# venomouscyanide/S3GRL

Hardware: AMD Instinct MI355X
Metric: link-pair precomputes/sec (higher is better)
Workload: dtype f32; 1 GPU; pubmed_pos_k3; mode=pos, sign_k=3, num_hops=3, num_nodes=19717, features=500, graph=real topology, synthetic features (BASELINE.md §3)

## Files before the change

### s3grl_amd/csrc/s3grl_api.hip

```cpp
#include <algorithm>
#include <chrono>
#include <cstdlib>
#include <cstring>
#include <memory>

#include "s3grl_internal.hpp"

namespace s3grl {

static thread_local std::string g_last_error;
void set_last_error(const std::string& msg) { g_last_error = msg; }

Arena::~Arena() {
  for (auto& kv : free_)
    if (!carved_.count(kv.second)) (void)hipFree(kv.second);
  for (auto& kv : live_)
    if (!carved_.count(kv.first)) (void)hipFree(kv.first);
  for (auto& sl : slabs_)
    if (sl.base) (void)hipFree(sl.base);
}

s3grl_status Arena::reserve(size_t bytes) {
  if (bytes < (1u << 20) || cached_ * 2 >= bytes) return S3GRL_OK;
  if (cur_slab_ >= 0 && slabs_[cur_slab_].size - slabs_[cur_slab_].used >= bytes) return S3GRL_OK;
// ... 731 lines not shown
      g_walk.balls = g->balls;
      S3GRL_TRY(launch_count_balls(ctx, &g_walk, links_walk, L, cfg->num_hops, plus ? 1 : 0, K, partner, mirror_of,
                                   plan->n_nodes, p_nodes, n_rows, n_jobs, lvl_max, reinterpret_cast<int32_t*>(ds),
                                   st + 3 * kStatRow, stash, slot, plan->lvl, perm));
    } else {
      S3GRL_TRY(launch_count(ctx, &g_walk, links_walk, L, cfg->num_hops, plus ? 1 : 0, K, ws,
                             partner, mirror_of,
                             plan->n_nodes, p_nodes, n_rows, n_jobs, lvl_max,
                             reinterpret_cast<int32_t*>(ds), st + 3 * kStatRow, smp, stash, slot, plan->lvl, perm));
    }
  }
  if (fold) S3GRL_TRY(launch_mirror_rows(ctx, partner, L, n_rows));
  S3GRL_TRY(launch_scan3(ctx, plan->n_nodes, n_rows, n_jobs, L, plan->node_off, plan->row_ptr, plan->job_off,
                         scan_ws, ds + 1, ds + 5, ds + 9));
  const bool csr_plan = !sop2 && !(cfg->flags & S3GRL_FLAG_COUNT_ONLY) && stash != nullptr && balls &&
                        csr_mode_for(g, cfg->num_hops, K, balls, relabel && !walks && !sampling && !onehop);
  if (!plus && !csr_plan)
    S3GRL_TRY(launch_classify(ctx, g, 1, K, plan->n_nodes, p_nodes, lvl_max, L, class_count, class_list,
                              !sampling && !g->directed, e_cap, stash ? slot : 0, perm, x_cap, nullptr, true));
  S3GRL_HIP_TRY(hipMemcpyAsync(hs, ds, 56 * 8, hipMemcpyDeviceToHost, ctx->stream));
  S3GRL_HIP_TRY(hipMemcpyAsync(ctx->h_stats + 3 * kStatRow, st + 3 * kStatRow, 2 * kStatRow * sizeof(int64_t),
                               hipMemcpyDeviceToHost, ctx->stream));
  S3GRL_HIP_TRY(hipStreamSynchronize(ctx->stream));
  hs[16] = hs[9];
  hs[17] = hs[10];
  hs[18] = hs[11];
  const int err = (int)(hs[0] & 0xffffffff);
  if (err == 2) {
    set_last_error("a link has src == dst");
    return S3GRL_ERR_SELF_LINK;
  }
  if (err == 1) {
    set_last_error("a link endpoint is outside [0, num_nodes)");
    return S3GRL_ERR_INVALID_ARGUMENT;
  }
  const int64_t max_n = hs[1], max_R = hs[5];
  const int64_t tot_n = hs[16], tot_rows = hs[17], njobs = hs[18];
  const int cn_cap = ((int)std::max<int64_t>(max_R - 2, 0) + 1) * ((relabel && plus) ? 3 : 1);
  uint16_t* csr_cnt = nullptr;
  int32_t* csr_e = nullptr;
  if (csr_plan) {
    S3GRL_TRY(arena_alloc(ctx, (size_t)std::max<int64_t>(tot_n, 1), &csr_cnt, tr));
    S3GRL_TRY(arena_alloc(ctx, (size_t)L, &csr_e, tr));
    S3GRL_TRY(launch_csr_count(ctx, &g_walk, links_walk, L, cfg->num_hops, plan->n_nodes, plan->node_off, plan->lvl,
                               stash, slot, perm, csr_cnt, csr_e));
  }
  if (plus || csr_plan) {
    S3GRL_TRY(launch_classify(ctx, g, plus ? cn_cap : 1, K, plan->n_nodes, p_nodes, lvl_max, L, class_count,
                              class_list, !sampling && !g->directed, e_cap, stash ? slot : 0, perm, x_cap, csr_e,
                              !plus));
    S3GRL_HIP_TRY(hipMemcpyAsync(hs + 32, ds + 32, 24 * 8, hipMemcpyDeviceToHost, ctx->stream));
    S3GRL_HIP_TRY(hipStreamSynchronize(ctx->stream));
  }
  int32_t class_count_host[48];
  std::memcpy(class_count_host, hs + 32, sizeof(class_count_host));
  if (getenv("S3GRL_DEBUG")) {
    fprintf(stderr, "[s3grl] L=%lld max_n=%lld classes:", (long long)L, (long long)max_n);
    for (int c = 0; c < num_class_lists(); ++c) fprintf(stderr, " %d", class_count_host[c]);
    fprintf(stderr, "\n");
  }
  if (cfg->flags & S3GRL_FLAG_COUNT_ONLY) {
    plan->stats.total_nodes = stat_total(3);
    plan->stats.folded_links = hs[7];
    plan->stats.extracted_nodes = tot_n;
    plan->stats.max_nodes = max_n;
    plan->stats.total_rows = tot_rows;
    plan->stats.num_row_pairs = 0;
    plan->njobs = 0;
    plan->stats.workspace_bytes = (int64_t)ctx->arena.bytes_held();
    *out = plan.release();
    return S3GRL_OK;
  }
  plan->stats.total_nodes = stat_total(3);
  plan->stats.oriented_entries = stat_total(4);
  plan->stats.folded_links = hs[7];
  plan->stats.extracted_nodes = tot_n;
  plan->stats.max_nodes = max_n;
  plan->stats.total_rows = tot_rows;
  plan->stats.num_row_pairs = njobs;
  plan->njobs = njobs;
  {
    int32_t* hist;
    S3GRL_TRY(arena_alloc(ctx, (size_t)256, &hist, tr));
    S3GRL_TRY(arena_alloc(ctx, (size_t)std::max<int64_t>(njobs, 1), &plan->job_order, own));
    int32_t* pc = nullptr;
    int64_t* po = nullptr;
    if (perm && hub_gather) {
      S3GRL_TRY(arena_alloc(ctx, (size_t)L, &pc, tr));
      S3GRL_TRY(arena_alloc(ctx, (size_t)(L + 1), &po, tr));
    }
    S3GRL_TRY(launch_job_order(ctx, plan->n_nodes, n_jobs, plan->job_off, L, hist, plan->job_order,
                               hub_gather ? perm : nullptr, pc, po, scan_ws));
  }
  plan->hub_order = perm != nullptr && hub_gather;

  const int64_t* coef_off = nullptr;
  int64_t tot_coef = tot_n;
  if (plus) {
    int32_t* job_n;
    int64_t* co;
    S3GRL_TRY(arena_alloc(ctx, (size_t)scan_workspace_elems(njobs), &scan_ws, tr));
    S3GRL_TRY(arena_alloc(ctx, (size_t)njobs, &job_n, tr));
    S3GRL_TRY(arena_alloc(ctx, (size_t)(njobs + 1), &co, tr));
    hipLaunchKernelGGL(expand_job_n_kernel, dim3((unsigned)((L + 255) / 256)), dim3(256), 0,
                       ctx->stream, plan->n_nodes, plan->job_off, L, job_n);
    S3GRL_HIP_TRY(hipGetLastError());
    S3GRL_TRY(launch_scan_i32_to_i64(ctx, job_n, njobs, co, scan_ws));
    S3GRL_HIP_TRY(hipMemcpyAsync(hs + 20, co + njobs, 8, hipMemcpyDeviceToHost, ctx->stream));
    S3GRL_HIP_TRY(hipStreamSynchronize(ctx->stream));
    tot_coef = hs[20];
    coef_off = co;
  }
  S3GRL_TRY(ctx->arena.reserve((size_t)std::max<int64_t>(tot_n, 1) * 4 + (size_t)std::max<int64_t>(tot_coef, 1) * 8 * K +
                               (size_t)njobs * (sizeof(Job) + 12 * K + 8) + (size_t)tot_rows * 8 + (16u << 20)));
  S3GRL_TRY(arena_alloc(ctx, (size_t)std::max<int64_t>(tot_n, 1), &plan->c_ids, own));
  S3GRL_TRY(arena_alloc(ctx, (size_t)std::max<int64_t>(tot_coef, 1) * 2 * K, &plan->c_coef, own));
  S3GRL_TRY(arena_alloc(ctx, (size_t)njobs, &plan->jobs, own));
  S3GRL_TRY(arena_alloc(ctx, (size_t)njobs * K * 2, &plan->job_z, own));
  S3GRL_TRY(arena_alloc(ctx, (size_t)std::max<int64_t>(njobs * K, 1), &plan->job_lim, own));
  S3GRL_TRY(arena_alloc(ctx, (size_t)tot_rows, &plan->row_nodes, own));
  int seg_shift = kSplitSegShift;
  if (const char* e = getenv("S3GRL_SPLIT_SEG_SHIFT")) seg_shift = std::min(20, std::max(4, atoi(e)));
  int split_t = kSplitThreshold;
  if (const char* e = getenv("S3GRL_SPLIT_T")) split_t = std::max(0, atoi(e));
  if (split_t > 0) split_t = std::max(split_t, 1 << seg_shift);
  if (max_n <= split_t) split_t = 0;
  plan->split_t = split_t;
  plan->seg_shift = seg_shift;
  S3GRL_TRY(record(ctx, 1));
  unsigned long long* tot = reinterpret_cast<unsigned long long*>(st);
  const LinkOut lo{plan->node_off, plan->row_ptr, plan->job_off, coef_off, mirror_of, plan->c_ids, plan->c_coef,
                    plan->jobs, plan->job_z, plan->job_lim, plan->row_nodes, plan->lvl, tot, tot + kStatRow,
                    tot + 2 * kStatRow, relabel ? g->old_of_new : nullptr, split_t, seg_shift};
  S3GRL_TRY(launch_links(ctx, &g_walk, links_walk, L, class_list, class_count_host, cfg->num_hops, plus ? 1 : 0,
                         cn_cap, (cfg->flags & S3GRL_FLAG_FULL_STATS) ? 1 : 0, K, ws, p_nodes, lo, smp, stash,
                         slot, e_cap, relabel ? g->new_of_old : nullptr, x_cap, csr_cnt, csr_e, sop2 ? 1 : 0));
  if (split_t > 0) {
    int32_t* pcnt;
    S3GRL_TRY(arena_alloc(ctx, (size_t)njobs, &pcnt, tr));
    S3GRL_TRY(arena_alloc(ctx, (size_t)(njobs + 1), &plan->piece_off, own));
    S3GRL_TRY(arena_alloc(ctx, (size_t)scan_workspace_elems(njobs), &scan_ws, tr));
    S3GRL_TRY(launch_split_count(ctx, plan->jobs, njobs, seg_shift, pcnt, plan->piece_off, scan_ws));
    S3GRL_HIP_TRY(hipMemcpyAsync(hs + 21, plan->piece_off + njobs, 8, hipMemcpyDeviceToHost, ctx->stream));
  }
  S3GRL_TRY(record(ctx, 2));
  S3GRL_HIP_TRY(hipMemcpyAsync(ctx->h_stats, st, 3 * kStatRow * sizeof(int64_t), hipMemcpyDeviceToHost,
                               ctx->stream));
  S3GRL_HIP_TRY(hipMemcpyAsync(ctx->h_stats + 4 * kStatRow, st + 4 * kStatRow, 5 * kStatRow * sizeof(int64_t),
                               hipMemcpyDeviceToHost, ctx->stream));
  plan->stats.workspace_bytes = (int64_t)ctx->arena.bytes_held();
  plan->stats_pending = true;
  ctx->stats_owner = plan.get();
  if (split_t > 0 || getenv("S3GRL_DEBUG_STAMPS")) {
    S3GRL_TRY(resolve_plan_stats(ctx));
    if (split_t > 0 && hs[21] > 0) {
      const int64_t np = hs[21];
      plan->npieces = np;
      const size_t units = (size_t)(njobs + np);
      S3GRL_TRY(arena_alloc(ctx, units, &plan->gjobs, own));
      S3GRL_TRY(arena_alloc(ctx, units * K * 2, &plan->g_z, own));
      S3GRL_TRY(arena_alloc(ctx, units * K, &plan->g_lim, own));
      S3GRL_TRY(arena_alloc(ctx, units, &plan->g_order, own));
      S3GRL_TRY(arena_alloc(ctx, (size_t)np, &plan->piece_job, own));
      S3GRL_HIP_TRY(hipMemcpyAsync(plan->g_z, plan->job_z, (size_t)njobs * K * 2 * sizeof(float),
                                   hipMemcpyDeviceToDevice, ctx->stream));
      S3GRL_HIP_TRY(hipMemsetAsync(plan->g_z + (size_t)njobs * K * 2, 0, (size_t)np * K * 2 * sizeof(float), ctx->stream));
      S3GRL_TRY(launch_split_fill(ctx, plan->jobs, plan->job_lim, njobs, plan->job_order, K, seg_shift,
                                  plan->piece_off, np, plan->gjobs, plan->g_lim, plan->g_order, plan->piece_job));
    }
    if (getenv("S3GRL_DEBUG_STAMPS")) {
      S3GRL_HIP_TRY(hipMemcpy(hs + 16, ds + 16, 8 * 8, hipMemcpyDeviceToHost));
      fprintf(stderr, "[s3grl] link_kernel phase cycles (sum over workgroups): bfs %lld  P/rank %lld  "
                      "deg %lld  ops<K %lld  last op %lld  tail %lld\n",
              (long long)hs[16], (long long)hs[17], (long long)hs[18], (long long)hs[19],
              (long long)hs[20], (long long)hs[21]);
      if (csr_plan)
        fprintf(stderr, "[s3grl] link_csr_kernel phase cycles (same slots): bitmap+ranks+offsets %lld  ids+rows %lld  "
                        "columns %lld  passes %lld   links %lld, mean LDS %lld B\n",
                (long long)hs[16], (long long)hs[17], (long long)hs[18], (long long)hs[19], (long long)hs[20],
                (long long)(hs[21] / std::max<int64_t>(hs[20], 1)));
      if (x_cap)
        fprintf(stderr, "[s3grl] link_hub_kernel phase cycles (same slots): nodes %lld  ids+rows %lld  walk %lld  "
                        "small csr %lld  passes %lld  tail %lld\n",
                (long long)hs[16], (long long)hs[17], (long long)hs[18], (long long)hs[19], (long long)hs[20],
                (long long)hs[21]);
      S3GRL_HIP_TRY(hipMemcpy(hs + 24, ds + 24, 8 * 8, hipMemcpyDeviceToHost));
      fprintf(stderr, "[s3grl] link_full_kernel, big class: merge %lld  hash+ids %lld  probes %lld  "
                      "csr+sort %lld  passes %lld   links %lld, columns in HBM for %lld\n",
              (long long)hs[24], (long long)hs[25], (long long)hs[26], (long long)hs[27], (long long)hs[28],
              (long long)hs[30], (long long)hs[31]);
    }
  }
  *out = plan.release();
  return S3GRL_OK;
}

s3grl_status s3grl_context_trim(s3grl_context* ctx, int64_t* released) {
  if (!ctx) return S3GRL_ERR_INVALID_ARGUMENT;
  S3GRL_HIP_TRY(hipSetDevice(ctx->device));
  S3GRL_HIP_TRY(hipStreamSynchronize(ctx->stream));
  for (auto& st : ctx->side)
    if (st) S3GRL_HIP_TRY(hipStreamSynchronize(st));
  const size_t freed = ctx->arena.trim();
  if (released) *released = (int64_t)freed;
  return S3GRL_OK;
}

s3grl_status s3grl_plan_gather_traffic(s3grl_context* ctx, const s3grl_plan* p,
                                       const s3grl_features* f, int64_t* what) {
  if (!ctx || !p || !f || !what) return S3GRL_ERR_INVALID_ARGUMENT;
  S3GRL_HIP_TRY(hipSetDevice(ctx->device));
  for (int i = 0; i < 8; ++i) what[i] = 0;
  if (p->njobs == 0) return S3GRL_OK;
  if (f->N != p->graph->num_nodes) return S3GRL_ERR_INVALID_ARGUMENT;
  S3GRL_HIP_TRY(hipMemsetAsync(ctx->d_scalars, 0, 8 * sizeof(int64_t), ctx->stream));
  S3GRL_TRY(launch_gather_traffic(ctx, p, f, reinterpret_cast<unsigned long long*>(ctx->d_scalars)));
  S3GRL_HIP_TRY(hipMemcpyAsync(ctx->h_scalars, ctx->d_scalars, 8 * sizeof(int64_t), hipMemcpyDeviceToHost,
                               ctx->stream));
  S3GRL_HIP_TRY(hipStreamSynchronize(ctx->stream));
  for (int i = 0; i < 8; ++i) what[i] = ctx->h_scalars[i];
  return S3GRL_OK;
}

s3grl_status s3grl_plan_get_stats(const s3grl_plan* p, s3grl_plan_stats* out) {
  if (!p || !out) return S3GRL_ERR_INVALID_ARGUMENT;
  if (p->stats_pending && p->ctx->stats_owner == p) S3GRL_TRY(resolve_plan_stats(p->ctx));
  *out = p->stats;
  return S3GRL_OK;
}

s3grl_status s3grl_plan_total_rows(const s3grl_plan* p, int64_t* total_rows) {
  if (!p || !total_rows) return S3GRL_ERR_INVALID_ARGUMENT;
  *total_rows = p->stats.total_rows;
  return S3GRL_OK;
}

s3grl_status s3grl_plan_counts(const s3grl_plan* p, int64_t* what) {
  if (!p || !what) return S3GRL_ERR_INVALID_ARGUMENT;
  what[0] = p->L;
  what[1] = p->stats.total_rows;
  what[2] = p->stats.folded_links;
  what[3] = p->njobs;
  return S3GRL_OK;
}

s3grl_status s3grl_plan_link_cost(const s3grl_plan* p, float* cost) {
  if (!p || (!cost && p->L)) return S3GRL_ERR_INVALID_ARGUMENT;
  if (p->L == 0) return S3GRL_OK;
  hipLaunchKernelGGL(link_cost_kernel, dim3((unsigned)((p->L + 255) / 256)), dim3(256), 0, p->ctx->stream,
                     p->n_nodes, p->e_cap, p->x_cap, p->row_ptr, p->L, kHubCostSlope, cost);
  S3GRL_HIP_TRY(hipGetLastError());
  return S3GRL_OK;
}

s3grl_status s3grl_plan_row_ptr(const s3grl_plan* p, int64_t* row_ptr) {
  if (!p || !row_ptr) return S3GRL_ERR_INVALID_ARGUMENT;
  S3GRL_HIP_TRY(hipMemcpyAsync(row_ptr, p->row_ptr, (size_t)(p->L + 1) * 8, hipMemcpyDeviceToDevice,
                               p->ctx->stream));
  return S3GRL_OK;
}

s3grl_status s3grl_plan_row_nodes(const s3grl_plan* p, int64_t* row_nodes) {
  if (!p || (!row_nodes && p->stats.total_rows)) return S3GRL_ERR_INVALID_ARGUMENT;
  if (p->stats.total_rows)
    S3GRL_HIP_TRY(hipMemcpyAsync(row_nodes, p->row_nodes, (size_t)p->stats.total_rows * 8,
                                 hipMemcpyDeviceToDevice, p->ctx->stream));
  return S3GRL_OK;
}

s3grl_status s3grl_plan_export_subgraphs(const s3grl_plan* p, int64_t* node_ptr, int32_t* nodes,
                                         int8_t* dists) {
  if (!p || !node_ptr) return S3GRL_ERR_INVALID_ARGUMENT;
  hipStream_t st = p->ctx->stream;
  S3GRL_HIP_TRY(hipMemcpyAsync(node_ptr, p->node_off, (size_t)(p->L + 1) * 8,
                               hipMemcpyDeviceToDevice, st));
  const size_t n = (size_t)p->stats.extracted_nodes;
  if ((nodes || dists) && (p->cfg.flags & S3GRL_FLAG_COUNT_ONLY)) {
    set_last_error("a count-only plan holds sizes only (pass NULL for nodes and dists)");
    return S3GRL_ERR_INVALID_ARGUMENT;
  }
  if (nodes && n) S3GRL_HIP_TRY(hipMemcpyAsync(nodes, p->c_ids, n * 4, hipMemcpyDeviceToDevice, st));
  if (nodes && n && p->relabelled) S3GRL_TRY(launch_sort_hops(p->ctx, p, nodes));
  if (dists && n) S3GRL_TRY(launch_dists(p->ctx, p->node_off, p->lvl, p->L, dists));
  return S3GRL_OK;
}

static s3grl_status run_with(s3grl_context* ctx, const s3grl_plan* p, const s3grl_features* f,
                             float* rows) {
  if (p->cfg.flags & S3GRL_FLAG_COUNT_ONLY) {
    set_last_error("a count-only plan cannot be run");
    return S3GRL_ERR_INVALID_ARGUMENT;
  }
  if (p->njobs == 0) return S3GRL_OK;
  if (f->N != p->graph->num_nodes) {
    set_last_error("features have " + std::to_string(f->N) + " rows, the graph " +
                   std::to_string(p->graph->num_nodes) + " nodes");
    return S3GRL_ERR_INVALID_ARGUMENT;
  }
  if (ctx->profiling) S3GRL_TRY(resolve_pending_gather(ctx));
  S3GRL_TRY(record(ctx, 3));
  auto gather = [&](const GatherView& v) -> s3grl_status {
    if (f->sparse) return launch_gather_sparse(ctx, p, v, f, rows);
    if (f->packed) return launch_gather_packed(ctx, p, v, f, rows);
    return launch_gather(ctx, v, p->c_ids, p->c_coef, p->cfg.sign_k, f->dense, f->ld, f->F, rows, p->hub_order);
  };
  if (p->npieces == 0) {
    S3GRL_TRY(gather(GatherView{p->jobs, p->njobs, p->job_z, p->job_lim, p->job_order, nullptr}));
  } else {
    Transient tmp{ctx, {}};
    void* q = nullptr;
    S3GRL_TRY(ctx->arena.alloc((size_t)p->npieces * 2 * (p->cfg.sign_k + 1) * (f->F + 1) * sizeof(float), &q));
    tmp.ptrs.push_back(q);
    float* prows = static_cast<float*>(q);
    S3GRL_TRY(gather(GatherView{p->gjobs, p->njobs + p->npieces, p->g_z, p->g_lim, p->g_order, prows}));
    S3GRL_TRY(launch_combine(ctx, p, prows, f->dense, f->ld, f->F, rows));
  }
  S3GRL_TRY(record(ctx, 4));
  if (ctx->profiling) ctx->gather_pending = true;
  return S3GRL_OK;
}

s3grl_status s3grl_run_features(s3grl_context* ctx, const s3grl_plan* p, const s3grl_features* f,
                                float* rows) {
  if (!ctx || !p || !f || (p->stats.total_rows && !rows)) return S3GRL_ERR_INVALID_ARGUMENT;
  S3GRL_HIP_TRY(hipSetDevice(ctx->device));
  return run_with(ctx, p, f, rows);
}

s3grl_status s3grl_run(s3grl_context* ctx, const s3grl_plan* p, const float* X, int64_t ldx,
                       int64_t F, float* rows) {
  if (!ctx || !p) return S3GRL_ERR_INVALID_ARGUMENT;
  if (!X) {
    set_last_error("node features are None");
    return S3GRL_ERR_NO_FEATURES;
  }
  if (F <= 0 || ldx < F || (p->stats.total_rows && !rows)) return S3GRL_ERR_INVALID_ARGUMENT;
  if (p->njobs == 0) return S3GRL_OK;
  s3grl_features* f = nullptr;
  S3GRL_TRY(s3grl_features_create(ctx, X, ldx, p->graph->num_nodes, F, 1, &f));
  const s3grl_status st = run_with(ctx, p, f, rows);
  s3grl_features_destroy(f);
  return st;
}

}

S3GRL_DEFINE_TOUCH(api)
```

### s3grl_amd/csrc/s3grl_csr.hip

```cpp
#include <hip/hip_runtime.h>

#include <algorithm>
#include <cstdlib>

#include "s3grl_device.hpp"

namespace s3grl {
namespace {

constexpr int kCsrCountT = 128;
constexpr int kCsrCountUn = 4;

__global__ __launch_bounds__(kCsrCountT) void csr_count_kernel(
    const int32_t* __restrict__ indptr, const int32_t* __restrict__ indices, int W, const uint32_t* __restrict__ balls,
    const int64_t* __restrict__ links, int hops, const int32_t* __restrict__ n_nodes,
    const int64_t* __restrict__ node_off, const int32_t* __restrict__ lvl, const int32_t* __restrict__ stash, int slot,
    const int32_t* __restrict__ perm, uint16_t* __restrict__ cnt, int32_t* __restrict__ csr_e) {
  extern __shared__ uint32_t smem[];
  constexpr int T = kCsrCountT;
  uint32_t* vis = smem;
  int* sh = reinterpret_cast<int*>(vis + W);
  const int tid = threadIdx.x;
  const int l = perm ? perm[blockIdx.x] : (int)blockIdx.x;
  const int n = n_nodes[l];
  if (n == 0 || n - 2 > slot) {
    if (tid == 0) csr_e[l] = -1;
    return;
  }
  const int src = (int)links[2 * (int64_t)l], dst = (int)links[2 * (int64_t)l + 1];
  const int64_t noff = node_off[l];
  const int32_t* lv = lvl + (int64_t)l * kMaxLevels;
  const int nlev = lv[kMaxLevels - 1];
  const int walk_from = nlev - 1 == hops ? lv[hops - 1] : n;
  const uint32_t* __restrict__ bs = balls + (int64_t)src * W;
  const uint32_t* __restrict__ bd = balls + (int64_t)dst * W;
  for (int w = tid; w < W; w += T) vis[w] = bs[w] | bd[w];
  const int32_t* __restrict__ st = stash + (int64_t)l * slot;
  const int32_t* list = st + (walk_from - 2);
  int e_local = 0;
  for (int t = tid; t < walk_from; t += T) {
    const int v = t < 2 ? (t == 0 ? min(src, dst) : max(src, dst)) : st[t - 2];
    const int b = indptr[v], d = indptr[v + 1] - b;
    int c = d;
    if (v == src || v == dst) c -= sorted_contains(indices + b, d, v == src ? dst : src) ? 1 : 0;
    cnt[noff + t] = (uint16_t)c;
    e_local += c;
  }
  __syncthreads();
  walk_rows<T, 4, kCsrCountUn>(
      0, n - walk_from, list, indptr, indices, nullptr,
      [&](RowAcc& a, int v, int u, bool valid) {
        const int mp = v == src ? dst : (v == dst ? src : -1);
        a.n += (valid && test_bit(vis, u) && u != mp) ? 1 : 0;
      },
      [&](RowAcc& a, int t, int) {
        cnt[noff + walk_from + t] = (uint16_t)a.n;
        e_local += a.n;
      });
  e_local = block_sum<T>(e_local, sh);
  if (tid == 0) csr_e[l] = e_local <= 65535 ? e_local : -1;
}

template <int T>
__global__ __launch_bounds__(T) void link_csr_kernel(const CsrLinkArgs a, const int32_t* __restrict__ class_list,
                                                     const int K) {
  extern __shared__ uint32_t smem[];
  constexpr int G = 4, RPI = T / G;
  const int32_t* __restrict__ indptr = a.indptr;
  const int32_t* __restrict__ indices = a.indices;
  const LinkOut& out = a.out;
  const int tid = threadIdx.x;
  const int l = class_list[blockIdx.x];
  const int64_t noff = out.node_off[l];
  const int n = (int)(out.node_off[l + 1] - noff);
  const int e = a.csr_e[l];
  const int W = a.W;
  const int mirror = out.mirror_of ? out.mirror_of[l] : -1;
  const int64_t mrp = mirror >= 0 ? out.row_ptr[mirror] : -1;

  int32_t* cn = reinterpret_cast<int32_t*>(smem);
  int32_t* cnpos = cn + a.cn_cap;
  int* lvl_end = cnpos + a.cn_cap;
  float* zbuf = reinterpret_cast<float*>(lvl_end + kMaxLevels);
  int* sh = reinterpret_cast<int*>(zbuf + 4 * K);
  float* dtab = reinterpret_cast<float*>(sh + 32);
  uint16_t* off = reinterpret_cast<uint16_t*>(dtab + kCsrDinvTable);
  uint16_t* cols = off + ((n + 2) & ~1);
  char* ubase = reinterpret_cast<char*>(smem) +
                (((reinterpret_cast<char*>(cols + ((e + 1) & ~1)) - reinterpret_cast<char*>(smem)) + 7) & ~(size_t)7);
  uint32_t* vis = reinterpret_cast<uint32_t*>(ubase);
  uint32_t* wpre = vis + W;
  int32_t* gb = reinterpret_cast<int32_t*>(wpre + W);
  uint16_t* gdeg = reinterpret_cast<uint16_t*>(gb + n);
  uint16_t* por = gdeg + ((n + 1) & ~1);
  float2* cur = reinterpret_cast<float2*>(ubase);
  float2* nxs = cur + n;

  unsigned long long t_prev = a.dbg ? __builtin_amdgcn_s_memtime() : 0ull;
  const int src = (int)a.links[2 * (int64_t)l], dst = (int)a.links[2 * (int64_t)l + 1];
  const int pos_src = src < dst ? 0 : 1, pos_dst = 1 - pos_src;
  const int32_t* lv = out.lvl + (int64_t)l * kMaxLevels;
  const int nlev = lv[kMaxLevels - 1];
  if (tid < nlev) lvl_end[tid] = lv[tid];
  for (int d = tid; d < kCsrDinvTable; d += T) dtab[d] = d > 0 ? 1.0f / sqrtf((float)d) : 0.0f;
  {
    const uint32_t* __restrict__ bs = a.balls + (int64_t)src * W;
    const uint32_t* __restrict__ bd = a.balls + (int64_t)dst * W;
    for (int w = tid; w < W; w += T) vis[w] = bs[w] | bd[w];
  }
  __syncthreads();
  {
    const int CW = (W + T - 1) / T, CN = (n + T - 1) / T;
    const int w0 = min(tid * CW, W), w1 = min(w0 + CW, W);
    const int t0 = min(tid * CN, n), t1 = min(t0 + CN, n);
    int pop = 0, cnt = 0;
    for (int w = w0; w < w1; ++w) pop += __popc(vis[w]);
    for (int t = t0; t < t1; ++t) cnt += a.cnt[noff + t];
    int total;
    const int run = block_excl_scan<T>((pop << 16) | cnt, sh, total);
    int rp_ = run >> 16, ro = run & 0xffff;
    for (int w = w0; w < w1; ++w) {
      wpre[w] = rp_;
      rp_ += __popc(vis[w]);
    }
    for (int t = t0; t < t1; ++t) {
      off[t] = (uint16_t)ro;
      ro += a.cnt[noff + t];
    }
    if (tid == 0) off[n] = (uint16_t)(total & 0xffff);
  }
  __syncthreads();
  phase_stamp(a.dbg, 0, t_prev);
  int vol_local = 0;
  {
    const int32_t* __restrict__ st = a.stash + (int64_t)l * a.slot;
    for (int t0 = tid; t0 < n; t0 += 4 * T) {
      int v[4], b[4], en[4];
#pragma unroll
      for (int k = 0; k < 4; ++k) {
        const int t = min(t0 + k * T, n - 1);
        v[k] = t < 2 ? (t == 0 ? min(src, dst) : max(src, dst)) : st[t - 2];
      }
#pragma unroll
      for (int k = 0; k < 4; ++k) {
        b[k] = indptr[(uint32_t)v[k]];
        en[k] = indptr[(uint32_t)v[k] + 1u];
      }
#pragma unroll
      for (int k = 0; k < 4; ++k) {
        const int t = t0 + k * T;
        if (t < n) {
          out.c_ids[noff + t] = ext_id(out, v[k]);
          vol_local += en[k] - b[k];
          gb[t] = b[k];
          gdeg[t] = (uint16_t)(en[k] - b[k]);
          por[rank_of(vis, wpre, v[k])] = (uint16_t)t;
        }
      }
    }
  }
  const int64_t rp = out.row_ptr[l];
  const int R = (int)(out.row_ptr[l + 1] - rp);
  const LinkSlot ls{l, src, dst, mirror, noff, rp, mrp};
  if (a.plus && wave_id() == 0) {
    auto in_s = [&](int u) -> bool { return test_bit(vis, u); };
    const int c = common_neighbours(indptr, indices, in_s, src, dst, cn);
    sort_caller_order(cn, c, out.old_of_new, lane_id());
  }
  __syncthreads();
  for (int r = tid; r < R; r += T) {
    const int node = row_node(r, src, dst, cn);
    write_row_node(out, ls, r, node);
    if (r >= 2) cnpos[r - 2] = por[rank_of(vis, wpre, node)];
  }
  if (tid == 0)
    for (int d = 0; d < kMaxLevels; ++d) export_level(out, l, d, nlev, lvl_end[d], n);

  phase_stamp(a.dbg, 1, t_prev);
  {
    const int g = tid & (G - 1);
    const int nib_shift = (tid & 63) & ~(G - 1);
    for (int base = 0; base < n; base += 2 * RPI) {
      int c0[2], e1[2], wc[2], mp[2], nx[2];
#pragma unroll
      for (int u = 0; u < 2; ++u) {
        const int t = base + u * RPI + tid / G;
        const bool ok = t < n;
        const int b = gb[min(t, n - 1)];
        c0[u] = ok ? b + g : 0;
        e1[u] = ok ? b + (int)gdeg[min(t, n - 1)] : 0;
        wc[u] = off[min(t, n)];
        mp[u] = t == pos_src ? dst : (t == pos_dst ? src : -1);
      }
#pragma unroll
      for (int u = 0; u < 2; ++u) nx[u] = indices[(uint32_t)(c0[u] < e1[u] ? c0[u] : 0)];
      while (__any(c0[0] < e1[0] || c0[1] < e1[1])) {
#pragma unroll
        for (int u = 0; u < 2; ++u) {
          const bool valid = c0[u] < e1[u];
          const int uu = nx[u];
          const int cnx = c0[u] + G;
          uint32_t an = (uint32_t)(cnx < e1[u] ? cnx : 0);
          asm volatile("" : "+v"(an));
          nx[u] = indices[an];
          const uint32_t bit = 1u << (uu & 31);
          const uint32_t wv = vis[uu >> 5];
          const int r = (int)wpre[uu >> 5] + __popc(wv & (bit - 1u));
          const int col = por[min(r, n - 1)];
          const bool member = valid && (wv & bit) && uu != mp[u];
          const unsigned nib = (unsigned)(__ballot(member) >> nib_shift) & ((1u << G) - 1u);
          if (member) cols[wc[u] + __popc(nib & ((1u << g) - 1u))] = (uint16_t)col;
          wc[u] += __popc(nib);
          c0[u] = cnx;
        }
      }
    }
  }
  __syncthreads();
  phase_stamp(a.dbg, 2, t_prev);

  auto dinv_of = [&](int t) -> float {
    const int d = (int)off[t + 1] - (int)off[t];
    return d < kCsrDinvTable ? dtab[d] : 1.0f / sqrtf((float)d);
  };
  const int npairs = (R + 1) / 2;
  for (int pr = 0; pr < npairs; ++pr) {
    const int64_t jid = out.job_off[l] + pr;
    const int64_t coff = out.coef_off ? out.coef_off[jid] : noff;
    int node_a, node_b, pos_a, pos_b;
    pair_rows(pr, R, src, dst, cn, node_a, node_b);
    pair_rows(pr, R, pos_src, pos_dst, cnpos, pos_a, pos_b);
    const int row_hop = pr == 0 ? 0 : 1;
    const int support = lvl_end[min(K + row_hop, nlev - 1)];
    for (int w = tid; w < n; w += T) {
      cur[w] = make_float2(0.f, 0.f);
      nxs[w] = make_float2(0.f, 0.f);
    }
    if (tid < 4 * K) zbuf[tid] = 0.f;
    __syncthreads();
    if (tid == 0) {
      cur[pos_a].x = dinv_of(pos_a);
      if (pos_b >= 0) cur[pos_b].y = dinv_of(pos_b);
    }
    __syncthreads();
    float2* s_in = cur;
    float2* s_out = nxs;
    float2* coef = reinterpret_cast<float2*>(out.c_coef) + coff * K;
    const bool split = split_list(out, support);
    auto cidx = [&](int i, int t) -> int64_t { return coef_index(i, t, support, K, split, out.seg_shift); };
#pragma unroll 1
    for (int i = 0; i < K; ++i) {
      const bool last = i == K - 1;
      const int limit = last ? support : lvl_end[min(i + 1 + row_hop, nlev - 1)];
      const int g = tid & (G - 1);
      for (int base = 0; base < limit; base += RPI) {
        const int t = base + tid / G;
        const bool ok = t < limit;
        const int b = ok ? (int)off[t] : 0, en = ok ? (int)off[t + 1] : 0;
        float ax = 0.f, ay = 0.f;
        for (int c = b + g; c < en; c += 2 * G) {
          const bool vb = c + G < en;
          const int ca = cols[c], cb = cols[vb ? c + G : c];
          const float2 sa = s_in[ca], sb = s_in[cb];
          ax += sa.x;
          ay += sa.y;
          ax += vb ? sb.x : 0.f;
          ay += vb ? sb.y : 0.f;
        }
#pragma unroll
        for (int o = G / 2; o > 0; o >>= 1) {
          ax += __shfl_xor(ax, o);
          ay += __shfl_xor(ay, o);
        }
        if (ok && g == 0) {
          const int d = en - b;
          const float dw = d < kCsrDinvTable ? dtab[d] : 1.0f / sqrtf((float)d);
          const float rx = dw * ax, ry = dw * ay;
          if (!last) s_out[t] = make_float2(dw * rx, dw * ry);
          coef[cidx(i, t)] = make_float2(rx, ry);
          if (t == pos_src) { zbuf[(0 * K + i) * 2] = rx; zbuf[(0 * K + i) * 2 + 1] = ry; }
          if (t == pos_dst) { zbuf[(1 * K + i) * 2] = rx; zbuf[(1 * K + i) * 2 + 1] = ry; }
        }
      }
      if (!last)
        for (int t = limit + tid; t < support; t += T) coef[cidx(i, t)] = make_float2(0.f, 0.f);
      __syncthreads();
      float2* tmp = s_in;
      s_in = s_out;
      s_out = tmp;
    }
    write_label_column(out, tid, K, jid, zbuf);
    end_pair(out, ls, tid, K, pr, jid, coff, support, node_a, node_b, split,
             [&](int i) { return i == K - 1 ? support : lvl_end[min(i + 1 + row_hop, nlev - 1)]; });
    __syncthreads();
  }
  phase_stamp(a.dbg, 3, t_prev);
  vol_local = block_sum<T>(vol_local, sh);
  if (tid == 0) {
    if (a.dbg) {
      atomicAdd(&a.dbg[4], 1ull);
      atomicAdd(&a.dbg[5], (unsigned long long)(4 * csr_fixed_words(a.cn_cap, K) + csr_lds_need(n, e, W)));
    }
    commit_link_stats(out, mirror, e, vol_local);
  }
}

}

int csr_class_bound(int cls, int cn_cap, int K) {
  static const int nominal[kCsrClasses] = S3GRL_CSR_CLASS_BOUNDS;
  const int avail = 163840 - 4 * csr_fixed_words(cn_cap, K);
  return cls == kCsrClasses - 1 ? avail : std::min(nominal[cls], avail);
}

bool csr_mode_for(const s3grl_graph* g, int hops, int K, bool balls, bool plain) {
  if (!balls || !plain || g->directed || getenv("S3GRL_NO_CSR")) return false;
  if (K - 1 < hops || hops < 1) return false;
  if (g->max_degree > kHubArmDegree) return false;
  if (getenv("S3GRL_FORCE_CSR")) return g->num_nodes <= 65536;
  return !sparse_mode_for(g) && g->num_nodes > 8192;
}

s3grl_status launch_csr_count(s3grl_context* ctx, const s3grl_graph* g, const int64_t* links, int64_t L, int hops,
                              const int32_t* n_nodes, const int64_t* node_off, const int32_t* lvl,
                              const int32_t* stash, int slot, const int32_t* perm, uint16_t* cnt, int32_t* csr_e) {
  if (L == 0) return S3GRL_OK;
  const int W = (int)((g->num_nodes + 31) / 32);
  const size_t lds = (size_t)4 * (W + 32);
  S3GRL_HIP_TRY(hipFuncSetAttribute(reinterpret_cast<const void*>(csr_count_kernel),
                                    hipFuncAttributeMaxDynamicSharedMemorySize, (int)lds));
  hipLaunchKernelGGL(csr_count_kernel, dim3((unsigned)L), dim3(kCsrCountT), lds, ctx->stream, g->indptr, g->indices, W,
                     g->balls.bits + (int64_t)(hops - 1) * g->balls.level_stride, links, hops, n_nodes, node_off, lvl,
                     stash, slot, perm, cnt, csr_e);
  S3GRL_HIP_TRY(hipGetLastError());
  return S3GRL_OK;
}

s3grl_status launch_csr_class(s3grl_context* ctx, const CsrLinkArgs& a, int K, int cls, const int32_t* class_list,
                              int count, hipStream_t stream) {
  if (count == 0) return S3GRL_OK;
  const size_t lds = (size_t)4 * csr_fixed_words(a.cn_cap, K) + (size_t)csr_class_bound(cls, a.cn_cap, K);
  const int t = lds <= 18 * 1024 ? 128 : (lds <= 26 * 1024 ? 256 : (lds <= 80 * 1024 ? 512 : 1024));
  auto go = [&](auto kern, int T) -> s3grl_status {
    S3GRL_HIP_TRY(hipFuncSetAttribute(reinterpret_cast<const void*>(kern), hipFuncAttributeMaxDynamicSharedMemorySize,
                                      (int)lds));
    hipLaunchKernelGGL(kern, dim3((unsigned)count), dim3(T), lds, stream, a, class_list, K);
    S3GRL_HIP_TRY(hipGetLastError());
    return S3GRL_OK;
  };
  if (t <= 128) return go(link_csr_kernel<128>, 128);
  if (t <= 256) return go(link_csr_kernel<256>, 256);
  if (t <= 512) return go(link_csr_kernel<512>, 512);
  return go(link_csr_kernel<1024>, 1024);
}

}

S3GRL_DEFINE_TOUCH(csr)
```

### s3grl_amd/csrc/s3grl_features.hip

```cpp
#include <algorithm>
#include <cstdlib>
#include <memory>

#include "s3grl_internal.hpp"
#include "s3grl_device.hpp"

namespace s3grl {
namespace {

constexpr int kTileCols = 512;

struct Entry {
  int32_t col;
  float val;
};

template <bool EVEN>
__global__ __launch_bounds__(256) void sp_count_kernel(const float* __restrict__ X, int64_t ldx,
                                                       int64_t N, int F, int tiles,
                                                       int32_t* __restrict__ cnt) {
  const int lane = threadIdx.x & 63;
  const int64_t item = (int64_t)blockIdx.x * 4 + (threadIdx.x >> 6);
  if (item >= N * tiles) return;
  const int tile = (int)(item / N);
  const int64_t row = item - (int64_t)tile * N;
  const int c0 = tile * kTileCols, c1 = min(F, c0 + kTileCols);
  int n = 0;
  for (int c = c0 + lane; c - lane < c1; c += 64) {
    const bool nz = c < c1 && X[row * ldx + c] != 0.f;
    n += __popcll(__ballot(nz));
  }
  if (lane == 0) cnt[item] = EVEN ? (n + 1) & ~1 : n;
}

__global__ __launch_bounds__(256) void sp_fill_kernel(const float* __restrict__ X, int64_t ldx,
                                                      int64_t N, int F, int tiles,
                                                      const int64_t* __restrict__ ptr,
                                                      Entry* __restrict__ ent) {
  const int lane = threadIdx.x & 63;
  const int64_t item = (int64_t)blockIdx.x * 4 + (threadIdx.x >> 6);
  if (item >= N * tiles) return;
  const int tile = (int)(item / N);
  const int64_t row = item - (int64_t)tile * N;
  const int c0 = tile * kTileCols, c1 = min(F, c0 + kTileCols);
  int64_t o = ptr[item];
  for (int c = c0 + lane; c - lane < c1; c += 64) {
    const float v = c < c1 ? X[row * ldx + c] : 0.f;
    const bool nz = v != 0.f;
    const unsigned long long m = __ballot(nz);
    if (nz) {
      Entry e;
      e.col = c - c0;
      e.val = v;
      ent[o + __popcll(m & ((1ull << lane) - 1ull))] = e;
    }
    o += __popcll(m);
  }
}

__global__ __launch_bounds__(256) void el_fill_kernel(const float* __restrict__ X, int64_t ldx, int64_t N, int F,
                                                      int tiles, const int64_t* __restrict__ ptr,
                                                      ElemEntry* __restrict__ ent, PackedHdr* __restrict__ hdr) {
  const int lane = threadIdx.x & 63;
  const int64_t item = (int64_t)blockIdx.x * 4 + (threadIdx.x >> 6);
  if (item >= N * tiles) return;
  const int tile = (int)(item / N);
  const int64_t row = item - (int64_t)tile * N;
  const int c0 = tile * kTileCols;
  uint32_t nzm = 0;
  if (lane < 32) {
    for (int m = 0; m < kTileCols / 32; ++m) {
      const int c = c0 + lane + 32 * m;
      if (c < F && X[row * ldx + c] != 0.f) nzm |= 1u << m;
    }
  }
  const int n = __popc(nzm);
  int total = n;
#pragma unroll
  for (int o = 32; o > 0; o >>= 1) total += __shfl_xor(total, o);
  const int h = (min(total, 64) + 1) / 2;
  const int64_t start = ptr[item];
  int o = 0;
  for (int r = 0;; ++r) {
    const unsigned long long bal = __ballot(n > r);
    if (bal == 0) break;
    if (n > r) {
      const int m = __ffs(nzm) - 1;
      nzm &= nzm - 1;
      ElemEntry e;
      e.slot = (uint32_t)(lane + 32 * m + 1);
      e.val = X[row * ldx + c0 + lane + 32 * m];
      const int q = o + __popcll(bal & ((1ull << lane) - 1ull));
      ent[start + (q >= 64 ? q : q < h ? 2 * q : 2 * (q - h) + 1)] = e;
    }
    o += __popcll(bal);
  }
  if (lane == 0) {
    if (total & 1) {
      ElemEntry e;
      e.slot = 0u;
      e.val = 0.f;
      ent[start + total] = e;
    }
    hdr[item].el = ((uint64_t)(uint32_t)total << 32) | (uint64_t)(uint32_t)start;
  }
}

__global__ void copy_pad_kernel(const float* __restrict__ X, int64_t ldx, int64_t N, int64_t F,
                                float* __restrict__ Y, int64_t ldy) {
  const int64_t total = N * ldy;
  for (int64_t i = (int64_t)blockIdx.x * blockDim.x + threadIdx.x; i < total;
       i += (int64_t)gridDim.x * blockDim.x) {
    const int64_t r = i / ldy, c = i - r * ldy;
    Y[i] = c < F ? X[r * ldx + c] : 0.f;
  }
}

template <int K>
__device__ __forceinline__ void scatter_entry(float2* acc, int col, float val, const float2* q) {
#pragma unroll
  for (int i = 0; i < K; ++i) {
    float2 a = acc[col * K + i];
    a.x += q[i].x * val;
    a.y += q[i].y * val;
    acc[col * K + i] = a;
  }
}

template <int K>
__global__ __launch_bounds__(256) void gather_sparse_kernel(
    const Job* __restrict__ jobs, int njobs, const int32_t* __restrict__ c_ids,
    const float* __restrict__ c_coef, const float* __restrict__ job_z,
    const int64_t* __restrict__ xptr, const Entry* __restrict__ ent, const float* __restrict__ X,
    int64_t ldx, int64_t N, int F, float* __restrict__ rows_out, float* __restrict__ prows) {
  extern __shared__ float2 lds2[];
  const int lane = threadIdx.x & 63;
  const int wave = threadIdx.x >> 6;
  const int jid = __builtin_amdgcn_readfirstlane(blockIdx.x * 4 + wave);
  if (jid >= njobs) return;
  float2* acc = lds2 + wave * (K * kTileCols);
  const int tile = blockIdx.y;
  const int col0 = tile * kTileCols;
  const int width = min(kTileCols, F - col0);
  const Job job = jobs[jid];
  if (job.split == 1) return;
  float* __restrict__ rows = job.split == 2 ? prows : rows_out;
  const int cnt = __builtin_amdgcn_readfirstlane(job.support);
  const int32_t* __restrict__ ids = c_ids + job.ids_off;
  const float2* __restrict__ cf = reinterpret_cast<const float2*>(c_coef) + job.coef_off;
  const int64_t* __restrict__ xp = xptr + (int64_t)tile * N;

  {
    float4* a4 = reinterpret_cast<float4*>(acc);
    for (int k = lane; k < K * kTileCols / 2; k += 64) a4[k] = make_float4(0.f, 0.f, 0.f, 0.f);
  }

  constexpr int U = 4;
  int j = 0;
  for (; j + U <= cnt; j += U) {
    int64_t beg[U], end[U];
    Entry e[U];
#pragma unroll
    for (int u = 0; u < U; ++u) {
      const int id = ids[j + u];
      beg[u] = xp[id];
      end[u] = xp[id + 1];
    }
#pragma unroll
    for (int u = 0; u < U; ++u) {
      e[u].col = 0;
      e[u].val = 0.f;
      if (beg[u] + lane < end[u]) e[u] = ent[beg[u] + lane];
    }
#pragma unroll
    for (int u = 0; u < U; ++u) {
      float2 q[K];
#pragma unroll
      for (int i = 0; i < K; ++i) q[i] = cf[(int64_t)i * cnt + j + u];
      if (beg[u] + lane < end[u]) scatter_entry<K>(acc, e[u].col, e[u].val, q);
      for (int64_t p = beg[u] + 64 + lane; p - lane < end[u]; p += 64) {
        if (p < end[u]) {
          const Entry t = ent[p];
          scatter_entry<K>(acc, t.col, t.val, q);
        }
      }
    }
  }
  for (; j < cnt; ++j) {
    const int id = ids[j];
    const int64_t b = xp[id], en = xp[id + 1];
    float2 q[K];
#pragma unroll
    for (int i = 0; i < K; ++i) q[i] = cf[(int64_t)i * cnt + j];
    for (int64_t p = b + lane; p - lane < en; p += 64) {
      if (p < en) {
        const Entry t = ent[p];
        scatter_entry<K>(acc, t.col, t.val, q);
      }
    }
  }

  const int Fp = F + 1;
  const int64_t rstride = (int64_t)(K + 1) * Fp;
  const int nrow = job.node_b >= 0 ? 2 : 1;
  const int ncopy = job.mirror_row >= 0 ? 2 : 1;
  for (int r = 0; r < nrow; ++r) {
    const int node = r == 0 ? job.node_a : job.node_b;
    const float* __restrict__ xr = X + (int64_t)node * ldx + col0;
    for (int m = 0; m < ncopy; ++m) {
      const int64_t orow = m == 0 ? job.out_row + r
                                  : job.mirror_row + (job.mirror_swap ? 1 - r : r);
      float* __restrict__ out = rows + orow * rstride;
      for (int c = lane; c < width; c += 64) {
        out[1 + col0 + c] = xr[c];
#pragma unroll
        for (int i = 0; i < K; ++i) {
          const float2 a = acc[c * K + i];
          out[(int64_t)(i + 1) * Fp + 1 + col0 + c] = r == 0 ? a.x : a.y;
        }
      }
      if (tile == 0 && lane <= K) {
        const float z = lane == 0 ? (float)(r == 0 ? job.z_a : job.z_b)
                                  : job_z[((int64_t)jid * K + (lane - 1)) * 2 + r];
        out[(int64_t)lane * Fp] = z;
      }
    }
  }
}

template <int K>
s3grl_status launch_sparse_k(s3grl_context* ctx, const s3grl_plan* p, const GatherView& v,
                             const s3grl_features* f, float* rows) {
  const unsigned gx = (unsigned)((v.njobs + 3) / 4);
  const size_t lds = (size_t)4 * 2 * K * kTileCols * sizeof(float);
  auto kern = gather_sparse_kernel<K>;
  S3GRL_HIP_TRY(hipFuncSetAttribute(reinterpret_cast<const void*>(kern),
                                    hipFuncAttributeMaxDynamicSharedMemorySize, (int)lds));
  hipLaunchKernelGGL(kern, dim3(gx, (unsigned)f->tiles), dim3(256), lds, ctx->stream, v.jobs,
                     (int)v.njobs, p->c_ids, p->c_coef, v.job_z, f->sp_ptr,
                     reinterpret_cast<const Entry*>(f->sp_ent), f->dense, f->ld, f->N, (int)f->F, rows, v.prows);
  S3GRL_HIP_TRY(hipGetLastError());
  return S3GRL_OK;
}

}

s3grl_status launch_copy_pad(s3grl_context* ctx, const float* X, int64_t ldx, int64_t N, int64_t F,
                             float* Y, int64_t ldy) {
  const int64_t total = N * ldy;
  if (total == 0) return S3GRL_OK;
  const unsigned grid = (unsigned)std::min<int64_t>((total + 255) / 256, 256 * 32);
  hipLaunchKernelGGL(copy_pad_kernel, dim3(grid), dim3(256), 0, ctx->stream, X, ldx, N, F, Y, ldy);
  S3GRL_HIP_TRY(hipGetLastError());
  return S3GRL_OK;
}

s3grl_status build_element_rows(s3grl_context* ctx, s3grl_features* f) {
  const int64_t N = f->N;
  const int64_t items = N * f->tiles;
  Transient tmp{ctx, {}};
  void* q = nullptr;
  S3GRL_TRY(ctx->arena.alloc((size_t)items * 4, &q));
  tmp.ptrs.push_back(q);
  int32_t* cnt = static_cast<int32_t*>(q);
  S3GRL_TRY(ctx->arena.alloc((size_t)(items + 1) * 8, &q));
  tmp.ptrs.push_back(q);
  int64_t* ptr = static_cast<int64_t*>(q);
  S3GRL_TRY(ctx->arena.alloc((size_t)scan_workspace_elems(items) * 8, &q));
  tmp.ptrs.push_back(q);
  int64_t* ws = static_cast<int64_t*>(q);
  const unsigned grid = (unsigned)((items + 3) / 4);
  hipLaunchKernelGGL(sp_count_kernel<true>, dim3(grid), dim3(256), 0, ctx->stream, f->dense, f->ld, N, (int)f->F,
                     f->tiles, cnt);
  S3GRL_HIP_TRY(hipGetLastError());
  S3GRL_TRY(launch_scan_i32_to_i64(ctx, cnt, items, ptr, ws));
  S3GRL_HIP_TRY(hipMemcpyAsync(ctx->h_scalars, ptr + items, 8, hipMemcpyDeviceToHost, ctx->stream));
  S3GRL_HIP_TRY(hipStreamSynchronize(ctx->stream));
  const int64_t nnz = ctx->h_scalars[0];
  if ((nnz + kTileCols) * (int64_t)sizeof(ElemEntry) >= ((int64_t)1 << 31)) return S3GRL_OK;
  S3GRL_TRY(ctx->arena.alloc((size_t)std::max<int64_t>(nnz, 1) * sizeof(ElemEntry), &q));
  f->owned.push_back(q);
  hipLaunchKernelGGL(el_fill_kernel, dim3(grid), dim3(256), 0, ctx->stream, f->dense, f->ld, N, (int)f->F, f->tiles,
                     ptr, static_cast<ElemEntry*>(q), const_cast<PackedHdr*>(static_cast<const PackedHdr*>(f->pk_hdr)));
  S3GRL_HIP_TRY(hipGetLastError());
  f->el_ent = q;
  f->el_nnz = nnz;
  f->elements = true;
  return S3GRL_OK;
}

s3grl_status launch_gather_sparse(s3grl_context* ctx, const s3grl_plan* p, const GatherView& v,
                                  const s3grl_features* f, float* rows) {
  if (v.njobs == 0) return S3GRL_OK;
  switch (p->cfg.sign_k) {
    case 1: return launch_sparse_k<1>(ctx, p, v, f, rows);
    case 2: return launch_sparse_k<2>(ctx, p, v, f, rows);
    case 3: return launch_sparse_k<3>(ctx, p, v, f, rows);
    case 4: return launch_sparse_k<4>(ctx, p, v, f, rows);
    case 5: return launch_sparse_k<5>(ctx, p, v, f, rows);
    case 6: return launch_sparse_k<6>(ctx, p, v, f, rows);
    case 7: return launch_sparse_k<7>(ctx, p, v, f, rows);
    case 8: return launch_sparse_k<8>(ctx, p, v, f, rows);
    default:
      set_last_error("sign_k must be in 1..8");
      return S3GRL_ERR_INVALID_ARGUMENT;
  }
}

}

using namespace s3grl;

extern "C" {

s3grl_status s3grl_features_destroy(s3grl_features* f) {
  if (!f) return S3GRL_OK;
  for (void* q : f->owned) f->ctx->arena.release(q);
  delete f;
  return S3GRL_OK;
}

s3grl_status s3grl_features_create(s3grl_context* ctx, const float* X, int64_t ldx, int64_t N,
                                   int64_t F, int32_t flags, s3grl_features** out) {
  if (!ctx || !out) return S3GRL_ERR_INVALID_ARGUMENT;
  if (!X) {
    set_last_error("node features are None");
    return S3GRL_ERR_NO_FEATURES;
  }
  if (N <= 0 || F <= 0 || ldx < F || F >= (int64_t)INT32_MAX / 2) return S3GRL_ERR_INVALID_ARGUMENT;
  S3GRL_HIP_TRY(hipSetDevice(ctx->device));
  std::unique_ptr<s3grl_features, s3grl_status (*)(s3grl_features*)> f(new s3grl_features(),
                                                                       s3grl_features_destroy);
  f->ctx = ctx;
  f->N = N;
  f->F = F;
  const int64_t need = (F + 3) / 4 * 4;
  if ((reinterpret_cast<uintptr_t>(X) & 15) == 0 && ldx % 4 == 0 && ldx >= need) {
    f->dense = X;
    f->ld = ldx;
  } else {
    void* p = nullptr;
    S3GRL_TRY(ctx->arena.alloc((size_t)N * need * 4, &p));
    f->owned.push_back(p);
    S3GRL_TRY(launch_copy_pad(ctx, X, ldx, N, F, static_cast<float*>(p), need));
    f->dense = static_cast<float*>(p);
    f->ld = need;
  }
  f->tiles = (int)((F + kTileCols - 1) / kTileCols);
  const bool no_elements = (flags & 8) != 0;
  flags &= ~8;
  if (flags != 2) {
    if (flags != 1) S3GRL_TRY(build_packed_rows(ctx, f.get(), flags == 4 ? 2.0 : 0.5, !no_elements));
    *out = f.release();
    return S3GRL_OK;
  }
  const int64_t items = N * f->tiles;
  int32_t* cnt = nullptr;
  int64_t *ptr = nullptr, *ws = nullptr;
  void* p = nullptr;
  S3GRL_TRY(ctx->arena.alloc((size_t)items * 4, &p));
  cnt = static_cast<int32_t*>(p);
  std::vector<void*> tmp{p};
  struct Rel {
    s3grl_context* c;
    std::vector<void*>* v;
    ~Rel() {
      for (void* q : *v) c->arena.release(q);
    }
  } rel{ctx, &tmp};
  S3GRL_TRY(ctx->arena.alloc((size_t)(items + 1) * 8, &p));
  ptr = static_cast<int64_t*>(p);
  tmp.push_back(ptr);
  S3GRL_TRY(ctx->arena.alloc((size_t)scan_workspace_elems(items) * 8, &p));
  ws = static_cast<int64_t*>(p);
  tmp.push_back(ws);
  hipLaunchKernelGGL(sp_count_kernel<false>, dim3((unsigned)((items + 3) / 4)), dim3(256), 0, ctx->stream,
                     f->dense, f->ld, N, (int)F, f->tiles, cnt);
  S3GRL_HIP_TRY(hipGetLastError());
  S3GRL_TRY(launch_scan_i32_to_i64(ctx, cnt, items, ptr, ws));
  S3GRL_HIP_TRY(hipMemcpyAsync(ctx->h_scalars, ptr + items, 8, hipMemcpyDeviceToHost, ctx->stream));
  S3GRL_HIP_TRY(hipStreamSynchronize(ctx->stream));
  f->nnz = ctx->h_scalars[0];
  const double density = (double)f->nnz / ((double)N * (double)F);
  (void)density;
  tmp.erase(std::find(tmp.begin(), tmp.end(), static_cast<void*>(ptr)));
  f->owned.push_back(ptr);
  f->sp_ptr = ptr;
  S3GRL_TRY(ctx->arena.alloc((size_t)std::max<int64_t>(f->nnz, 1) * sizeof(Entry), &p));
  f->owned.push_back(p);
  f->sp_ent = p;
  hipLaunchKernelGGL(sp_fill_kernel, dim3((unsigned)((items + 3) / 4)), dim3(256), 0, ctx->stream,
                     f->dense, f->ld, N, (int)F, f->tiles, ptr, static_cast<Entry*>(p));
  S3GRL_HIP_TRY(hipGetLastError());
  f->sparse = true;
  *out = f.release();
  return S3GRL_OK;
}

s3grl_status s3grl_features_info(const s3grl_features* f, int64_t* nnz, int32_t* is_sparse) {
  if (!f) return S3GRL_ERR_INVALID_ARGUMENT;
  if (nnz) *nnz = f->packed || !f->sparse ? f->pk_chunks : f->nnz;
  if (is_sparse) *is_sparse = f->sparse ? 1 : (f->packed ? 2 : 0);
  return S3GRL_OK;
}

}

S3GRL_DEFINE_TOUCH(features)
```

### s3grl_amd/csrc/s3grl_gather.hip

```cpp
#include <cstdlib>

#include "s3grl_internal.hpp"
#include "s3grl_gather_common.hpp"

namespace s3grl {
namespace {

constexpr int kWavesPerBlock = 4;
constexpr int kUnroll = 8;
constexpr int kNarrowUnroll = 8;

template <int K, int CH>
__global__ __launch_bounds__(kWavesPerBlock * 64) void gather_kernel(
    const Job* __restrict__ jobs, int njobs, const int32_t* __restrict__ c_ids,
    const float* __restrict__ c_coef, const float* __restrict__ job_z, const float* __restrict__ X,
    int64_t ldx, int F, float* __restrict__ rows_out, float* __restrict__ prows,
    const int32_t* __restrict__ job_order) {
  const int lane = threadIdx.x & 63;
  const int wid = __builtin_amdgcn_readfirstlane(blockIdx.x * kWavesPerBlock + (threadIdx.x >> 6));
  if (wid >= njobs) return;
  const int jid = job_order ? __builtin_amdgcn_readfirstlane(job_order[wid]) : wid;
  const int col0 = blockIdx.y * (CH * 256);
  const Job job = jobs[jid];
  if (job.split == 1) return;
  float* __restrict__ rows = job.split == 2 ? prows : rows_out;
  const int cnt = __builtin_amdgcn_readfirstlane(job.support);
  const int32_t* __restrict__ ids = c_ids + job.ids_off;
  const float2* __restrict__ cf = reinterpret_cast<const float2*>(c_coef) + job.coef_off;

  int coff[CH];
  bool cok[CH];
#pragma unroll
  for (int c = 0; c < CH; ++c) {
    coff[c] = col0 + (lane + 64 * c) * 4;
    cok[c] = coff[c] < F;
  }

  float4_t acc[K][2][CH];
#pragma unroll
  for (int i = 0; i < K; ++i)
#pragma unroll
    for (int r = 0; r < 2; ++r)
#pragma unroll
      for (int c = 0; c < CH; ++c) acc[i][r][c] = (float4_t)(0.f);

  int j = 0;
  for (; j + kUnroll <= cnt; j += kUnroll) {
    float4_t v[kUnroll][CH];
    int id[kUnroll];
#pragma unroll
    for (int u = 0; u < kUnroll; ++u) id[u] = ids[j + u];
#pragma unroll
    for (int u = 0; u < kUnroll; ++u) {
      const float* __restrict__ xr = X + (int64_t)id[u] * ldx;
#pragma unroll
      for (int c = 0; c < CH; ++c)
        v[u][c] = cok[c] ? *reinterpret_cast<const float4_t*>(xr + coff[c]) : (float4_t)(0.f);
    }
#pragma unroll
    for (int i = 0; i < K; ++i) {
#pragma unroll
      for (int u = 0; u < kUnroll; ++u) {
        const float2 q = cf[(int64_t)i * cnt + j + u];
#pragma unroll
        for (int c = 0; c < CH; ++c) {
          acc[i][0][c] += q.x * v[u][c];
          acc[i][1][c] += q.y * v[u][c];
        }
      }
    }
  }
  for (; j < cnt; ++j) {
    const float* __restrict__ xr = X + (int64_t)ids[j] * ldx;
#pragma unroll
    for (int c = 0; c < CH; ++c) {
      const float4_t v = cok[c] ? *reinterpret_cast<const float4_t*>(xr + coff[c]) : (float4_t)(0.f);
#pragma unroll
      for (int i = 0; i < K; ++i) {
        const float2 q = cf[(int64_t)i * cnt + j];
        acc[i][0][c] += q.x * v;
        acc[i][1][c] += q.y * v;
      }
    }
  }

  write_pair_rows<K, CH>(job, jid, acc, coff, cok, job_z, X, ldx, F, rows, blockIdx.y == 0);
}

typedef float float2_t __attribute__((ext_vector_type(2)));
typedef float float2_u __attribute__((ext_vector_type(2), aligned(4)));

template <int K>
__global__ __launch_bounds__(kWavesPerBlock * 64) void gather_narrow_kernel(
    const Job* __restrict__ jobs, int njobs, const int32_t* __restrict__ c_ids,
    const float* __restrict__ c_coef, const float* __restrict__ job_z, const float* __restrict__ X,
    int64_t ldx, int F, float* __restrict__ rows_out, float* __restrict__ prows,
    const int32_t* __restrict__ job_order) {
  constexpr int U = K <= 3 ? kNarrowUnroll : (K == 4 ? 6 : (K == 5 ? 5 : (K == 6 ? 4 : 3)));
  const int lane = threadIdx.x & 63;
  const int wid = __builtin_amdgcn_readfirstlane(blockIdx.x * kWavesPerBlock + (threadIdx.x >> 6));
  if (wid >= njobs) return;
  const int jid = job_order ? __builtin_amdgcn_readfirstlane(job_order[wid]) : wid;
  const Job job = jobs[jid];
  if (job.split == 1) return;
  float* __restrict__ rows = job.split == 2 ? prows : rows_out;
  const int cnt = __builtin_amdgcn_readfirstlane(job.support);
  const int32_t* __restrict__ ids = c_ids + job.ids_off;
  const float2* __restrict__ cf = reinterpret_cast<const float2*>(c_coef) + job.coef_off;
  const int coff = lane * 2;
  const bool col_ok = coff < F;
  const uint32_t voff = (uint32_t)(col_ok ? coff : 0) * 4u;
  float2_t acc[K][2];
#pragma unroll
  for (int i = 0; i < K; ++i) {
    acc[i][0] = (float2_t)(0.f);
    acc[i][1] = (float2_t)(0.f);
  }
  const uint32_t row_bytes = (uint32_t)ldx * 4u;
  auto row_of = [&](int id) -> float2_t {
    uint64_t prod = (uint64_t)(uint32_t)id * row_bytes;
    asm volatile("" : "+s"(prod));
    const char* base = reinterpret_cast<const char*>(X) + prod;
    uint32_t vo = voff;
    asm volatile("" : "+v"(vo));
    return *reinterpret_cast<const float2_t*>(base + vo);
  };
  const int nrow = job.node_b >= 0 ? 2 : 1;
  const int ng = cnt / U;
  if (ng > 0) {
    int id[U];
#pragma unroll
    for (int u = 0; u < U; ++u) id[u] = ids[u];
    for (int g = 0; g < ng; ++g) {
      float2_t v[U];
#pragma unroll
      for (int u = 0; u < U; ++u) v[u] = row_of(id[u]);
      __builtin_amdgcn_sched_barrier(0);
      const int jn = min(g + 1, ng - 1) * U;
#pragma unroll
      for (int u = 0; u < U; ++u) id[u] = ids[jn + u];
      float2 q[K][U];
#pragma unroll
      for (int i = 0; i < K; ++i)
#pragma unroll
        for (int u = 0; u < U; ++u) q[i][u] = cf[(int64_t)i * cnt + g * U + u];
      __builtin_amdgcn_sched_barrier(0);
#pragma unroll
      for (int i = 0; i < K; ++i) {
#pragma unroll
        for (int u = 0; u < U; ++u) {
          acc[i][0] += q[i][u].x * v[u];
          acc[i][1] += q[i][u].y * v[u];
        }
      }
      __builtin_amdgcn_sched_barrier(0);
    }
  }
  for (int j = ng * U; j < cnt; ++j) {
    const float2_t v = row_of(ids[j]);
#pragma unroll
    for (int i = 0; i < K; ++i) {
      const float2 q = cf[(int64_t)i * cnt + j];
      acc[i][0] += q.x * v;
      acc[i][1] += q.y * v;
    }
  }
  const int Fp = F + 1;
  const int64_t rstride = (int64_t)(K + 1) * Fp;
  const int ncopy = job.mirror_row >= 0 ? 2 : 1;
  const int nv = min(2, F - coff);
#pragma unroll
  for (int r = 0; r < 2; ++r) {
    if (r >= nrow) break;
    const float2_t x0 = row_of(r == 0 ? job.node_a : job.node_b);
    for (int m = 0; m < ncopy; ++m) {
      const int64_t orow = m == 0 ? job.out_row + r : job.mirror_row + (job.mirror_swap ? 1 - r : r);
      float* __restrict__ out = rows + orow * rstride;
      if (col_ok) {
        float* o = out + 1 + coff;
        if (nv == 2) {
          *reinterpret_cast<float2_u*>(o) = x0;
#pragma unroll
          for (int i = 0; i < K; ++i) *reinterpret_cast<float2_u*>(o + (int64_t)(i + 1) * Fp) = acc[i][r];
        } else {
          o[0] = x0[0];
#pragma unroll
          for (int i = 0; i < K; ++i) o[(int64_t)(i + 1) * Fp] = acc[i][r][0];
        }
      }
      if (lane <= K) {
        const float z = lane == 0 ? (float)(r == 0 ? job.z_a : job.z_b)
                                  : job_z[((int64_t)jid * K + (lane - 1)) * 2 + r];
        out[(int64_t)lane * Fp] = z;
      }
    }
  }
}

template <int K>
s3grl_status launch_k(s3grl_context* ctx, const Job* jobs, int64_t njobs, const int32_t* c_ids,
                      const float* c_coef, const float* job_z, const float* X, int64_t ldx,
                      int64_t F, float* rows, float* prows, const int32_t* job_order) {
  hipStream_t stream = ctx->stream;
  const unsigned gx = (unsigned)((njobs + kWavesPerBlock - 1) / kWavesPerBlock);
  if (F <= 128 && ldx < ((int64_t)1 << 30)) {
    hipLaunchKernelGGL((gather_narrow_kernel<K>), dim3(gx, 1), dim3(kWavesPerBlock * 64), 0, stream,
                       jobs, (int)njobs, c_ids, c_coef, job_z, X, ldx, (int)F, rows, prows, job_order);
  } else if (F <= 256) {
    hipLaunchKernelGGL((gather_kernel<K, 1>), dim3(gx, 1), dim3(kWavesPerBlock * 64), 0, stream,
                       jobs, (int)njobs, c_ids, c_coef, job_z, X, ldx, (int)F, rows, prows, job_order);
  } else {
    const unsigned gy = (unsigned)((F + 511) / 512);
    hipLaunchKernelGGL((gather_kernel<K, 2>), dim3(gx, gy), dim3(kWavesPerBlock * 64), 0,
                       stream, jobs, (int)njobs, c_ids, c_coef, job_z, X, ldx, (int)F, rows, prows, job_order);
  }
  S3GRL_HIP_TRY(hipGetLastError());
  return S3GRL_OK;
}

}

s3grl_status launch_gather(s3grl_context* ctx, const GatherView& v, const int32_t* c_ids,
                           const float* c_coef, int K, const float* X, int64_t ldx, int64_t F, float* rows,
                           bool in_job_order) {
  const Job* jobs = v.jobs;
  const int64_t njobs = v.njobs;
  const float* job_z = v.job_z;
  const int32_t* order = in_job_order ? v.job_order : nullptr;
  if (njobs == 0) return S3GRL_OK;
  switch (K) {
    case 1: return launch_k<1>(ctx, jobs, njobs, c_ids, c_coef, job_z, X, ldx, F, rows, v.prows, order);
    case 2: return launch_k<2>(ctx, jobs, njobs, c_ids, c_coef, job_z, X, ldx, F, rows, v.prows, order);
    case 3: return launch_k<3>(ctx, jobs, njobs, c_ids, c_coef, job_z, X, ldx, F, rows, v.prows, order);
    case 4: return launch_k<4>(ctx, jobs, njobs, c_ids, c_coef, job_z, X, ldx, F, rows, v.prows, order);
    case 5: return launch_k<5>(ctx, jobs, njobs, c_ids, c_coef, job_z, X, ldx, F, rows, v.prows, order);
    case 6: return launch_k<6>(ctx, jobs, njobs, c_ids, c_coef, job_z, X, ldx, F, rows, v.prows, order);
    case 7: return launch_k<7>(ctx, jobs, njobs, c_ids, c_coef, job_z, X, ldx, F, rows, v.prows, order);
    case 8: return launch_k<8>(ctx, jobs, njobs, c_ids, c_coef, job_z, X, ldx, F, rows, v.prows, order);
    default:
      set_last_error("sign_k must be in 1..8");
      return S3GRL_ERR_INVALID_ARGUMENT;
  }
}

}

S3GRL_DEFINE_TOUCH(gather)
```

### s3grl_amd/csrc/s3grl_gather_common.hpp

```cpp
#pragma once

#include "s3grl_internal.hpp"

namespace s3grl {
namespace {

typedef float float4_t __attribute__((ext_vector_type(4)));
typedef float float4_u __attribute__((ext_vector_type(4), aligned(4)));

template <int K, int CH, int I0, int I1, bool XROW, bool ZCOL>
__device__ __forceinline__ void write_pair_rows_part(const Job& job, int jid, const float4_t (&acc)[K][2][CH],
                                                     const int (&coff)[CH], const bool (&cok)[CH],
                                                     const float* __restrict__ job_z,
                                                     const float* __restrict__ X, int64_t ldx, int F,
                                                     float* __restrict__ rows, bool first_tile) {
  const int lane = threadIdx.x & 63;
  const int Fp = F + 1;
  const int64_t rstride = (int64_t)(K + 1) * Fp;
  const int nrow = job.node_b >= 0 ? 2 : 1;
  const int ncopy = job.mirror_row >= 0 ? 2 : 1;
#pragma unroll
  for (int r = 0; r < 2; ++r) {
    if (r >= nrow) break;
    const int node = r == 0 ? job.node_a : job.node_b;
    const float* __restrict__ xr = X + (int64_t)node * ldx;
    for (int m = 0; m < ncopy; ++m) {
      const int64_t orow = m == 0 ? job.out_row + r
                                  : job.mirror_row + (job.mirror_swap ? 1 - r : r);
      float* __restrict__ out = rows + orow * rstride;
#pragma unroll
      for (int c = 0; c < CH; ++c) {
        if (cok[c]) {
          const int nv = min(4, F - coff[c]);
          if constexpr (XROW) {
            const float4_t x0 = *reinterpret_cast<const float4_t*>(xr + coff[c]);
            float* o = out + 1 + coff[c];
            if (nv == 4) {
              *reinterpret_cast<float4_u*>(o) = x0;
            } else {
#pragma unroll
              for (int e = 0; e < 4; ++e)
                if (e < nv) o[e] = x0[e];
            }
          }
#pragma unroll
          for (int i = I0; i < I1; ++i) {
            const float4_t a = acc[i][r][c];
            float* oi = out + (int64_t)(i + 1) * Fp + 1 + coff[c];
            if (nv == 4) {
              *reinterpret_cast<float4_u*>(oi) = a;
            } else {
#pragma unroll
              for (int e = 0; e < 4; ++e)
                if (e < nv) oi[e] = a[e];
            }
          }
        }
      }
      if constexpr (ZCOL) {
        if (first_tile && lane <= K) {
          const float z = lane == 0 ? (float)(r == 0 ? job.z_a : job.z_b)
                                    : job_z[((int64_t)jid * K + (lane - 1)) * 2 + r];
          out[(int64_t)lane * Fp] = z;
        }
      }
    }
  }
}

template <int K, int CH>
__device__ __forceinline__ void write_pair_rows(const Job& job, int jid, const float4_t (&acc)[K][2][CH],
                                                const int (&coff)[CH], const bool (&cok)[CH],
                                                const float* __restrict__ job_z,
                                                const float* __restrict__ X, int64_t ldx, int F,
                                                float* __restrict__ rows, bool first_tile) {
  write_pair_rows_part<K, CH, 0, K, true, true>(job, jid, acc, coff, cok, job_z, X, ldx, F, rows, first_tile);
}

}
}
```

### s3grl_amd/csrc/s3grl_internal.hpp

```cpp
#pragma once

#include <hip/hip_runtime.h>

#include <cstdint>
#include <cstdio>
#include <map>
#include <string>
#include <vector>

#include "../../include/s3grl.h"

namespace s3grl {

void set_last_error(const std::string& msg);

#define S3GRL_HIP_TRY(expr)                                                                   \
  do {                                                                                        \
    hipError_t _e = (expr);                                                                   \
    if (_e != hipSuccess) {                                                                   \
      ::s3grl::set_last_error(std::string(#expr) + ": " + hipGetErrorString(_e) + " (" +      \
                              __FILE__ + ":" + std::to_string(__LINE__) + ")");               \
      return _e == hipErrorOutOfMemory ? S3GRL_ERR_OUT_OF_MEMORY : S3GRL_ERR_HIP;             \
    }                                                                                         \
  } while (0)

#define S3GRL_TRY(expr)                    \
  do {                                     \
    s3grl_status _s = (expr);              \
    if (_s != S3GRL_OK) return _s;         \
  } while (0)

constexpr int kBlock = 256;
constexpr int kMaxNodesLds = 327680;
constexpr int kMaxSignK = 8;
constexpr int kStatShards = 64;
constexpr int kStatStride = 16;
constexpr int kStatRows = 9;
constexpr int kMaxLevels = 32;
constexpr int kNumClasses = 6;

struct HopSampling {
  double ratio;
  int32_t max_nodes;
  uint32_t seed;
};
static inline bool hop_sampling_on(const HopSampling& s) {
  return (s.ratio > 0.0 && s.ratio < 1.0) || s.max_nodes > 0;
}

struct WalkSets {
  const int32_t* raw = nullptr;
  int len = 0;
  const int64_t* ptr = nullptr;
  const int32_t* nodes = nullptr;
  int per_link = 0;
  int num_nodes = 0;
};
__host__ __device__ static inline bool walks_on(const WalkSets& w) { return w.raw != nullptr || w.ptr != nullptr; }

struct Job {
  int64_t coef_off;
  int64_t ids_off;
  int64_t out_row;
  int32_t link;
  int32_t support;
  int32_t node_a;
  int32_t node_b;
  int32_t z_a;
  int32_t z_b;
  int64_t mirror_row;
  int32_t mirror_swap;
  int32_t split;
};

constexpr int kSplitThreshold = 4096;
constexpr int kSplitSegShift = 10;

__host__ __device__ __forceinline__ int64_t piece_coef_off(int s0, int K) { return (int64_t)s0 * K; }
__host__ __device__ __forceinline__ int64_t coef_index(int i, int t, int support, int K, bool split, int seg_shift) {
  if (!split) return (int64_t)i * support + t;
  const int s0 = (t >> seg_shift) << seg_shift;
  const int len = min(1 << seg_shift, support - s0);
  return piece_coef_off(s0, K) + (int64_t)i * len + (t - s0);
}

struct LinkOut {
  const int64_t *node_off, *row_ptr, *job_off;
  const int64_t* coef_off;
  const int32_t* mirror_of;
  int32_t* c_ids;
  float* c_coef;
  Job* jobs;
  float* job_z;
  int32_t* job_lim;
  int64_t* row_nodes;
  int32_t* lvl;
  unsigned long long *tot_edges, *tot_support, *tot_vol;
  const int32_t* old_of_new;
  int split_t, seg_shift;
};
constexpr int64_t kHubOrderMinNodes = 65536;
constexpr int64_t kHubOrderMinLinks = 65536;

struct GatherView {
  const Job* jobs;
  int64_t njobs;
  const float* job_z;
  const int32_t* job_lim;
  const int32_t* job_order;
  float* prows;
};

class Arena {
 public:
  ~Arena();
  s3grl_status alloc(size_t bytes, void** out);
  void release(void* p);
  size_t trim();
  size_t bytes_held() const { return held_; }
  s3grl_status reserve(size_t bytes);
  size_t cached_bytes() const { return cached_; }

 private:
  struct Slab {
    char* base;
    size_t size, used;
    int blocks;
  };
  std::multimap<size_t, void*> free_;
  std::map<void*, size_t> live_;
  std::map<void*, int> carved_;
  std::vector<Slab> slabs_;
  int cur_slab_ = -1;
  size_t held_ = 0, cached_ = 0;
};

}

struct s3grl_context {
  int device = 0;
  hipStream_t stream = nullptr;
  s3grl::Arena arena;
  bool profiling = false;
  bool gather_pending = false;
  double timings[16] = {0};
  hipEvent_t ev[8] = {nullptr, nullptr, nullptr, nullptr, nullptr, nullptr, nullptr, nullptr};
  static constexpr int kSide = 3;
  hipStream_t side[kSide] = {nullptr, nullptr, nullptr};
  hipEvent_t side_ev[kSide + 1] = {nullptr, nullptr, nullptr, nullptr};
  int64_t* d_scalars = nullptr;
  int64_t* h_scalars = nullptr;
  int64_t* d_stats = nullptr;
  int64_t* h_stats = nullptr;
  s3grl_plan* stats_owner = nullptr;
};

struct HubCache {
  int32_t nh = 0;
  int32_t* slot = nullptr;
  int32_t* voln = nullptr;
  int64_t* row_base = nullptr;
  int64_t* col_base = nullptr;
  int32_t* hoff = nullptr;
  uint16_t* hcols = nullptr;
};
constexpr int kHubMinDegree = 128;
constexpr int kHubClasses = 4;
constexpr int64_t kHubVolMax = 262144;

struct BallCache {
  int hops = 0;
  int64_t level_stride = 0;
  uint32_t* bits = nullptr;
};

struct s3grl_graph {
  s3grl_context* ctx = nullptr;
  HubCache hub;
  BallCache balls;
  int64_t num_nodes = 0;
  int64_t nnz = 0;
  int32_t max_degree = 0;
  int32_t* indptr = nullptr;
  int32_t* indices = nullptr;
  int32_t* fwd_indptr = nullptr;
  int32_t* fwd_indices = nullptr;
  uint16_t* fwd_deg = nullptr;
  int32_t* r_indptr = nullptr;
  int32_t* r_indices = nullptr;
  int32_t* new_of_old = nullptr;
  int32_t* old_of_new = nullptr;
  int32_t deg_le2_from = 0;
  int32_t* r_fwd_indptr = nullptr;
  int32_t* r_fwd_indices = nullptr;
  uint16_t* r_fwd_deg = nullptr;
  bool directed = false;
  int64_t arcs = 0;
  int32_t* out_indptr = nullptr;
  int32_t* out_indices = nullptr;
  int32_t* in_indptr = nullptr;
  int32_t* in_indices = nullptr;
};

struct DirGraph {
  const int32_t* out_indptr = nullptr;
  const int32_t* out_indices = nullptr;
  const int32_t* in_indptr = nullptr;
  const int32_t* in_indices = nullptr;
};

struct s3grl_plan {
  s3grl_context* ctx = nullptr;
  const s3grl_graph* graph = nullptr;
  s3grl_cfg cfg{};
  int64_t L = 0;
  s3grl_plan_stats stats{};
  int64_t* links = nullptr;
  int32_t* n_nodes = nullptr;
  int64_t* node_off = nullptr;
  int64_t* row_ptr = nullptr;
  int64_t* job_off = nullptr;
  int32_t* lvl = nullptr;
  int32_t* e_cap = nullptr;
  int64_t* x_cap = nullptr;
  bool relabelled = false;
  bool stats_pending = false;
  bool hub_order = false;
  bool walk_plan = false;
  int32_t* c_ids = nullptr;
  s3grl::Job* jobs = nullptr;
  int64_t njobs = 0;
  float* job_z = nullptr;
  int32_t* job_order = nullptr;
  int32_t* job_lim = nullptr;
  float* c_coef = nullptr;
  int64_t* row_nodes = nullptr;
  int split_t = 0, seg_shift = 0;
  int64_t npieces = 0;
  int64_t* piece_off = nullptr;
  s3grl::Job* gjobs = nullptr;
  float* g_z = nullptr;
  int32_t* g_lim = nullptr;
  int32_t* g_order = nullptr;
  int32_t* piece_job = nullptr;
  std::vector<void*> owned;
};

struct s3grl_features {
  s3grl_context* ctx = nullptr;
  int64_t N = 0, F = 0;
  const float* dense = nullptr;
  int64_t ld = 0;
  bool sparse = false;
  int tiles = 0;
  int64_t nnz = 0;
  const int64_t* sp_ptr = nullptr;
  const void* sp_ent = nullptr;
  bool packed = false;
  const void* pk_hdr = nullptr;
  const void* pk_data = nullptr;
  int64_t pk_chunks = 0;
  bool elements = false;
  const void* el_ent = nullptr;
  int64_t el_nnz = 0;
  std::vector<void*> owned;
};

struct PackedHdr {
  uint64_t m0, m1;
  uint64_t off;
  uint64_t el;
};

struct ElemEntry {
  float val;
  uint32_t slot;
};

struct s3grl_sop {
  s3grl_context* ctx = nullptr;
  const s3grl_graph* graph = nullptr;
  int32_t K = 0;
  int64_t F = 0;
  int64_t ldy = 0;
  const float* mult = nullptr;
  double* dinv = nullptr;
  double* Y = nullptr;
  float* Yhi = nullptr;
  float* Ylo = nullptr;
  std::vector<void*> owned;
};

#define S3GRL_DEFINE_TOUCH(unit)                                                               \
  namespace s3grl {                                                                            \
  namespace {                                                                                  \
  __global__ void touch_kernel_##unit() {}                                                     \
  }                                                                                            \
  void touch_##unit() {                                                                        \
    hipFuncAttributes at;                                                                      \
    (void)hipFuncGetAttributes(&at, reinterpret_cast<const void*>(touch_kernel_##unit));       \
  }                                                                                            \
  }

namespace s3grl {

void touch_api();
void touch_structure();
void touch_links_k12();
void touch_links_k34();
void touch_links_k56();
void touch_links_k78();
void touch_gather();
void touch_packed();
void touch_features();
void touch_sop();
void touch_pool();
void touch_relabel();
void touch_hub();
void touch_balls();
void touch_csr();

struct Transient {
  s3grl_context* ctx;
  std::vector<void*> ptrs;
  ~Transient() {
    for (void* p : ptrs) ctx->arena.release(p);
  }
};

s3grl_status ensure_side_streams(s3grl_context* ctx);

s3grl_status build_degree_order(s3grl_context* ctx, s3grl_graph* g);
s3grl_status launch_translate_links(s3grl_context* ctx, const s3grl_graph* g, const int64_t* links, int64_t L,
                                    int64_t* out);
s3grl_status launch_link_order(s3grl_context* ctx, const int64_t* links, int64_t L, int64_t N,
                               const int32_t* indptr, int32_t* perm);
s3grl_status sort_pairs_u64_i32_bytes(s3grl_context* ctx, size_t n, size_t* bytes);
s3grl_status sort_pairs_u64_i32(s3grl_context* ctx, void* tmp, size_t bytes, uint64_t* keys_in, uint64_t* keys_out,
                                int32_t* vals_in, int32_t* vals_out, size_t n);
struct SortScratch {
  void* tmp = nullptr;
  size_t bytes = 0;
};
s3grl_status sort_keys_u64_bytes(s3grl_context* ctx, size_t n, int end_bit, size_t* bytes);
s3grl_status sort_keys_u64(s3grl_context* ctx, SortScratch& scratch, uint64_t* keys_in, uint64_t* keys_out, size_t n,
                           int end_bit);
s3grl_status launch_epoch_perm(s3grl_context* ctx, uint64_t key, int64_t n, uint64_t* keys_a, uint64_t* keys_b,
                               SortScratch& scratch, int32_t* perm);
s3grl_status launch_init_normal(s3grl_context* ctx, uint64_t key, int64_t n, float* out);
s3grl_status launch_init_uniform(s3grl_context* ctx, uint64_t key, float bound, int64_t n, float* out);
s3grl_status launch_fill(s3grl_context* ctx, float value, int64_t n, float* out);
s3grl_status segmented_sort_i32(s3grl_context* ctx, void* tmp, size_t* bytes, const int32_t* keys_in, int32_t* keys_out,
                                size_t n, unsigned segments, const int64_t* seg);
s3grl_status ensure_ball_cache(s3grl_context* ctx, s3grl_graph* g, int hops, bool* usable);
void release_ball_cache(s3grl_graph* g);
s3grl_status launch_count_balls(s3grl_context* ctx, const s3grl_graph* g, const int64_t* links, int64_t L, int hops,
                                int plus, int K, const int32_t* partner, const int32_t* mirror_of, int32_t* n_nodes,
                                int32_t* p_nodes, int32_t* n_rows, int32_t* n_jobs, int32_t* lvl_max,
                                int32_t* err_flag, int64_t* tot_nodes_alg, int32_t* stash, int slot,
                                int32_t* lvl_stash, const int32_t* perm);
s3grl_status build_hub_cache(s3grl_context* ctx, s3grl_graph* g);
void release_hub_cache(s3grl_graph* g);
__host__ __device__ inline int64_t hub_lds_need(int64_t n, int64_t xcap) {
  const int64_t state = 16 * n, build = 4 * n + 4 * xcap;
  return 8 * n + 16 + (state > build ? state : build) + 4 * ((xcap + 1) & ~(int64_t)1) + 2 * ((n + 1) & ~(int64_t)1);
}
__host__ __device__ inline int64_t hub_stage_bytes(int64_t c, int64_t entries) {
  return entries <= 65535 ? 2 * ((c + 2) & ~(int64_t)1) + 2 * ((entries + 1) & ~(int64_t)1) : 0;
}
int hub_fixed_words(int cn_cap, int K);
int hub_class_bound(int cls, int cn_cap, int K);
struct HubLinkArgs {
  const int32_t *indptr, *indices;
  HubCache hub;
  const int64_t* links;
  int plus, cn_cap;
  const int64_t* x_cap;
  LinkOut out;
  unsigned long long *tot_oriented, *tot_hub_links, *tot_hub_bytes, *tot_hub_ends, *tot_hub_nodes;
  const int32_t* e_cap;
  unsigned long long* dbg;
  uint32_t* slices;
  int64_t slice_words;
  int slice_grid;
};
s3grl_status launch_hub_class(s3grl_context* ctx, const HubLinkArgs& a, int K, int cls, const int32_t* class_list,
                              int count, hipStream_t stream);
s3grl_status launch_sort_hops(s3grl_context* ctx, const s3grl_plan* p, int32_t* nodes);

constexpr int kTinyNodes = 64;
struct TinyLinkArgs {
  const int32_t *indptr, *indices, *fwd_indptr, *fwd_indices;
  const int64_t* links;
  LinkOut out;
};
s3grl_status launch_tiny_class(s3grl_context* ctx, const TinyLinkArgs& a, int K, int width, const int32_t* class_list,
                               int count, hipStream_t stream);

constexpr int kCsrBase = 32;
constexpr int kCsrClasses = 14;
#define S3GRL_CSR_CLASS_BOUNDS {4096, 6144, 8192, 12288, 16384, 20480, 24576, 32768, 40960, 49152, 65536, 98304, 131072, 163840}
struct CsrBounds {
  int b[kCsrClasses];
};
constexpr int kCsrDinvTable = 256;
__host__ __device__ inline int csr_fixed_words(int cn_cap, int K) {
  return 2 * cn_cap + kMaxLevels + 4 * K + 32 + kCsrDinvTable;
}
__host__ __device__ inline int csr_lds_need(int n, int e, int W) {
  const int off_b = 2 * ((n + 2) & ~1), col_b = 2 * ((e + 1) & ~1);
  const int build = 8 * W + 4 * n + 4 * ((n + 2) & ~1), pass = 16 * n;
  return ((off_b + col_b + 7) & ~7) + (build > pass ? build : pass) + 8;
}
struct CsrLinkArgs {
  const int32_t *indptr, *indices;
  int W, hops;
  const uint32_t* balls;
  const int64_t* links;
  int plus, cn_cap;
  const uint16_t* cnt;
  const int32_t* csr_e;
  LinkOut out;
  const int32_t* stash;
  int slot;
  unsigned long long* dbg;
};
int csr_class_bound(int cls, int cn_cap, int K);
bool csr_mode_for(const s3grl_graph* g, int hops, int K, bool balls, bool plain);
s3grl_status launch_csr_count(s3grl_context* ctx, const s3grl_graph* g_walk, const int64_t* links, int64_t L, int hops,
                              const int32_t* n_nodes, const int64_t* node_off, const int32_t* lvl,
                              const int32_t* stash, int slot, const int32_t* perm, uint16_t* cnt, int32_t* csr_e);
s3grl_status launch_csr_class(s3grl_context* ctx, const CsrLinkArgs& a, int K, int cls, const int32_t* class_list,
                              int count, hipStream_t stream);

s3grl_status launch_count(s3grl_context* ctx, const s3grl_graph* g, const int64_t* links, int64_t L,
                          int hops, int plus, int K, WalkSets ws,
                          const int32_t* partner, const int32_t* mirror_of, int32_t* n_nodes, int32_t* p_nodes,
                          int32_t* n_rows, int32_t* n_jobs, int32_t* lvl_max, int32_t* err_flag,
                          int64_t* tot_nodes_alg, HopSampling smp = HopSampling{1.0, 0, 0},
                          int32_t* stash = nullptr, int slot = 0, int32_t* lvl_stash = nullptr,
                          const int32_t* perm = nullptr);
s3grl_status build_union_graph(s3grl_context* ctx, int64_t N, const int32_t* a_indptr, const int32_t* a_indices,
                               const int32_t* b_indptr, const int32_t* b_indices, int32_t* u_indptr,
                               int32_t** u_indices, int64_t* u_nnz);
int num_class_lists();
s3grl_status launch_random_walks(s3grl_context* ctx, const s3grl_graph* g, int m, int M,
                                 uint32_t seed, int32_t* raw);
s3grl_status launch_validate_sets(s3grl_context* ctx, const int64_t* set_ptr, const int32_t* set_nodes,
                                  int64_t num_sets, int64_t total, int64_t num_nodes,
                                  int64_t* flags );
s3grl_status launch_walk_sets(s3grl_context* ctx, const s3grl_graph* g, const int64_t* starts, int64_t num_starts,
                              int m, int M, uint32_t seed, int64_t* set_ptr, int32_t* set_nodes);
int64_t mirror_table_slots(int64_t L);
s3grl_status launch_find_mirrors(s3grl_context* ctx, const int64_t* links, int64_t L, int64_t N,
                                 uint64_t* keys, int32_t* vals, int64_t slots, int32_t* partner,
                                 int32_t* mirror_of, int64_t* n_mirrored);
s3grl_status launch_mirror_rows(s3grl_context* ctx, const int32_t* partner, int64_t L,
                                int32_t* n_rows);
s3grl_status launch_job_order(s3grl_context* ctx, const int32_t* n_nodes, const int32_t* n_jobs,
                              const int64_t* job_off, int64_t L, int32_t* hist, int32_t* job_order,
                              const int32_t* perm = nullptr, int32_t* scratch_cnt = nullptr,
                              int64_t* scratch_off = nullptr, int64_t* scan_ws = nullptr);
int64_t scan_workspace_elems(int64_t n);
s3grl_status launch_scan_i32_to_i64(s3grl_context* ctx, const int32_t* in, int64_t n, int64_t* out,
                                    int64_t* workspace);
s3grl_status launch_scan3(s3grl_context* ctx, const int32_t* in0, const int32_t* in1, const int32_t* in2,
                          int64_t n, int64_t* out0, int64_t* out1, int64_t* out2, int64_t* workspace3,
                          int64_t* max0, int64_t* max1, int64_t* totals);
s3grl_status launch_classify(s3grl_context* ctx, const s3grl_graph* g, int cn_cap, int K,
                             const int32_t* n_nodes, const int32_t* p_nodes,
                             const int32_t* lvl_max, int64_t L, int32_t* class_count,
                             int32_t* class_list, bool allow_hash = true, const int32_t* e_cap = nullptr,
                             int stash_slot = 0, const int32_t* perm = nullptr, const int64_t* x_cap = nullptr,
                             const int32_t* csr_e = nullptr, bool tiny_ok = false);
bool sparse_mode_for(const s3grl_graph* g);
bool onehop_mode_for(const s3grl_graph* g);
s3grl_status build_forward_rows(s3grl_context* ctx, s3grl_graph* g);
s3grl_status launch_count1(s3grl_context* ctx, const s3grl_graph* g, const int64_t* links, int64_t L,
                           int plus, int K, const int32_t* partner, const int32_t* mirror_of,
                           int32_t* n_nodes, int32_t* p_nodes, int32_t* n_rows, int32_t* n_jobs,
                           int32_t* lvl_max, int32_t* e_cap, int32_t* err_flag, int64_t* tot_nodes_alg,
                           int64_t* tot_oriented, const int32_t* perm = nullptr, int64_t* x_cap = nullptr);
s3grl_status launch_links(s3grl_context* ctx, const s3grl_graph* g, const int64_t* links, int64_t L,
                          const int32_t* class_list, const int32_t* class_count_host, int hops,
                          int plus, int cn_cap, int full_stats, int K, WalkSets ws, const int32_t* p_nodes,
                          const LinkOut& out, HopSampling smp, const int32_t* stash, int slot,
                          const int32_t* e_cap, const int32_t* new_of_old, const int64_t* x_cap,
                          const uint16_t* csr_cnt, const int32_t* csr_e, int sop2);
s3grl_status launch_split_count(s3grl_context* ctx, const Job* jobs, int64_t njobs, int seg_shift,
                                int32_t* cnt, int64_t* piece_off, int64_t* scan_ws);
s3grl_status launch_split_fill(s3grl_context* ctx, const Job* jobs, const int32_t* job_lim, int64_t njobs,
                               const int32_t* job_order, int K, int seg_shift, const int64_t* piece_off,
                               int64_t npieces, Job* gjobs, int32_t* g_lim, int32_t* g_order, int32_t* piece_job);
s3grl_status launch_combine(s3grl_context* ctx, const s3grl_plan* p, const float* prows, const float* X,
                            int64_t ldx, int64_t F, float* rows);
s3grl_status launch_dists(s3grl_context* ctx, const int64_t* node_off, const int32_t* lvl, int64_t L,
                          int8_t* dists);
s3grl_status launch_gather(s3grl_context* ctx, const GatherView& v, const int32_t* c_ids,
                           const float* c_coef, int K, const float* X, int64_t ldx, int64_t F, float* rows,
                           bool in_job_order = false);
s3grl_status build_packed_rows(s3grl_context* ctx, s3grl_features* f, double max_density, bool elements);
s3grl_status build_element_rows(s3grl_context* ctx, s3grl_features* f);
s3grl_status launch_gather_packed(s3grl_context* ctx, const s3grl_plan* p, const GatherView& v,
                                  const s3grl_features* f, float* rows);
s3grl_status launch_gather_traffic(s3grl_context* ctx, const s3grl_plan* p, const s3grl_features* f,
                                   unsigned long long* d_out );
s3grl_status launch_gather_sparse(s3grl_context* ctx, const s3grl_plan* p, const GatherView& v,
                                  const s3grl_features* f, float* rows);
s3grl_status launch_copy_pad(s3grl_context* ctx, const float* X, int64_t ldx, int64_t N, int64_t F,
                             float* Y, int64_t ldy);

}
```

### s3grl_amd/csrc/s3grl_link_classes.hpp

```cpp
#pragma once

#include <algorithm>
#include <cstdlib>

#include "s3grl_internal.hpp"
#include "s3grl_device.hpp"

namespace s3grl {
namespace {

constexpr int kBmMaxNodes = 512;
__host__ __device__ __forceinline__ int link_bm_bytes(int n, int p) {
  return (p == n && n <= kBmMaxNodes) ? 4 * n * ((n + 31) >> 5) + 4 * n + 8 : 0;
}
__host__ __device__ __forceinline__ int link_lds_need(int n, int p) { return 4 * n + 20 * p + 16; }
__host__ __device__ __forceinline__ int link_lds_need_sparse(int n, int p) {
  int C = 64;
  while (C < 2 * n) C <<= 1;
  return 8 * C + link_lds_need(n, p) + link_bm_bytes(n, p);
}

struct ClassBounds {
  int b[kNumClasses];
};

constexpr int kSparseBase = kNumClasses + 2;
constexpr int kFullBase = kSparseBase + kNumClasses;
constexpr int kFullBig = kFullBase + kNumClasses;
constexpr int kHubBase = kFullBig + 1;
constexpr int kNumLists = kHubBase + kHubClasses + 1;
constexpr int kTinyList = kNumLists;
static_assert(kTinyList + 1 < 29, "class_count[29..31] carry maxima");
constexpr int kNumListsAll = kCsrBase + kCsrClasses;

__device__ __forceinline__ int row_lower_bound(const int32_t* __restrict__ a, int n, int x) {
  int lo = 0, hi = n;
  while (lo < hi) {
    const int mid = (lo + hi) >> 1;
    if (a[mid] < x) lo = mid + 1; else hi = mid;
  }
  return lo;
}

__host__ __device__ __forceinline__ int full_hash_slots(int n) {
  int C = 64;
  while (C < 2 * n) C <<= 1;
  return C;
}
__host__ __device__ __forceinline__ int full_lds_need(int n, int ecap, bool on_chip) {
  const int WB = (n + 31) >> 5;
  return 8 * full_hash_slots(n) + 12 * n + 16 + (on_chip ? 2 * ((ecap + 1) & ~1) + 4 * n * WB : 64 * WB);
}

constexpr int kLongRow = 96;
constexpr int kLongCap = 128;

}

static inline int words_for(int64_t N) { return (int)((N + 31) / 32); }

static inline int link_fixed_words(int64_t num_nodes, int cn_cap, int K) {
  return 3 * words_for(num_nodes) + cn_cap + kMaxLevels + 4 * K + 32 + kHubWords;
}
static inline int link_fixed_words_sparse(int cn_cap, int K) {
  return cn_cap + kMaxLevels + 4 * K + 32 + kHubWords;
}

static constexpr int kNominalBounds[kNumClasses] = {6144, 12288, 24576, 49152, 98304, 163840};

static ClassBounds class_bounds(int64_t num_nodes, int cn_cap, int K) {
  const int* nominal = kNominalBounds;
  int avail = 163840 - 4 * link_fixed_words(num_nodes, cn_cap, K);
  if (const char* e = getenv("S3GRL_LDS_BUDGET")) avail = std::min(avail, atoi(e));
  ClassBounds cb;
  for (int c = 0; c < kNumClasses; ++c) cb.b[c] = std::min(nominal[c], avail);
  cb.b[kNumClasses - 1] = avail;
  return cb;
}
static ClassBounds class_bounds_sparse(int cn_cap, int K) {
  static const int nominal[kNumClasses] = {4096, 8192, 16384, 32768, 65536, 131072};
  const int avail = 163840 - 4 * link_fixed_words_sparse(cn_cap, K);
  ClassBounds cb;
  for (int c = 0; c < kNumClasses; ++c) cb.b[c] = std::min(nominal[c], avail);
  return cb;
}

static inline int full_fixed_words(int cn_cap, int K) { return 2 * cn_cap + 2 + 4 * K + 32 + kLongCap / 2; }
static ClassBounds class_bounds_full(int cn_cap, int K) {
  static const int nominal[kNumClasses] = {3072, 6144, 12288, 24576, 65536, 160000};
  const int avail = 163840 - 4 * full_fixed_words(cn_cap, K);
  ClassBounds cb;
  for (int c = 0; c < kNumClasses; ++c) cb.b[c] = std::min(nominal[c], avail);
  return cb;
}

static int threads_for_class(size_t lds, int c) {
  if (c == 0 && lds <= 40 * 1024) return 128;
  return lds <= 40 * 1024 ? 256 : (lds <= 80 * 1024 ? 512 : 1024);
}

static inline int link_fixed_words_dm(int64_t num_nodes, int cn_cap, int K) {
  return 16 * words_for(num_nodes) + cn_cap + kMaxLevels + 4 * K + 32 + kHubWords;
}
static ClassBounds class_bounds_dm(int64_t num_nodes, int cn_cap, int K) {
  const int* nominal = kNominalBounds;
  const int avail = 163840 - 4 * link_fixed_words_dm(num_nodes, cn_cap, K);
  ClassBounds cb;
  for (int c = 0; c < kNumClasses; ++c) cb.b[c] = std::min(nominal[c], avail);
  cb.b[kNumClasses - 1] = avail;
  return cb;
}

static bool dm_mode_for(const s3grl_graph* g) {
  if (sparse_mode_for(g) || getenv("S3GRL_NO_DM")) return false;
  return g->num_nodes <= 8192;
}

static int waves_per_cu(size_t lds, int c) {
  return std::min<int>(32, (int)(163840 / std::max<size_t>(lds, 1)) * (threads_for_class(lds, c) / 64));
}
static int dm_class_mask_for(const s3grl_graph* g, int cn_cap, int K) {
  const ClassBounds bb = class_bounds(g->num_nodes, cn_cap, K), bd = class_bounds_dm(g->num_nodes, cn_cap, K);
  int mask = 0;
  for (int c = 0; c < kNumClasses; ++c) {
    if (bd.b[c] <= 0) continue;
    if (bb.b[c] <= 0) { mask |= 1 << c; continue; }
    const int wb = waves_per_cu((size_t)4 * link_fixed_words(g->num_nodes, cn_cap, K) + bb.b[c], c);
    const int wd = waves_per_cu((size_t)4 * link_fixed_words_dm(g->num_nodes, cn_cap, K) + bd.b[c], c);
    const size_t lb = (size_t)4 * link_fixed_words(g->num_nodes, cn_cap, K) + bb.b[c];
    const size_t ld = (size_t)4 * link_fixed_words_dm(g->num_nodes, cn_cap, K) + bd.b[c];
    if (c == 0 && 2 * std::min<size_t>(163840 / ld, 16) < std::min<size_t>(163840 / lb, 16)) continue;
    if (5 * wd >= 4 * wb) mask |= 1 << c;
  }
  return mask;
}

struct LinkArgs {
  const s3grl_graph* g;
  const int64_t* links;
  const int32_t* class_list;
  int hops, plus, cn_cap, full_stats;
  WalkSets ws;
  const int32_t* p_nodes;
  LinkOut out;
  char* scratch;
  int64_t scratch_stride;
  unsigned long long* dbg;
  HopSampling smp;
  const int32_t* stash;
  int slot;
  const int32_t* e_cap;
  uint32_t* bm_scratch;
  int64_t bm_stride_words;
  int bm_grid;
  int big_need;
  const int32_t* new_of_old;
  int lo_id;
  DirGraph dg;
  int bm_ext_words;
  int gs_chunk;
  int64_t list_offset;
  const int64_t* x_cap;
  uint32_t* hub_slices;
  int64_t hub_slice_words;
  int hub_slice_grid;
  const uint16_t* csr_cnt;
  const int32_t* csr_e;
  int sop2;
};

template <int K>
s3grl_status launch_links_k(s3grl_context* ctx, const LinkArgs& a, int64_t L, const int32_t* class_count_in);

}
```

### s3grl_amd/csrc/s3grl_packed.hip

```cpp
#include <algorithm>
#include <cstdlib>
#include <type_traits>

#include "s3grl_internal.hpp"
#include "s3grl_gather_common.hpp"

namespace s3grl {
namespace {


constexpr int kTile = 512;
constexpr int kWavesPerBlock = 1;
constexpr int kPrefixWindow = 64;
constexpr int kRecStride = 32;
constexpr int kStageDwords = kPrefixWindow / 4 * kRecStride + 64;

__device__ __forceinline__ int below(uint64_t m) {
  return __builtin_amdgcn_mbcnt_hi((uint32_t)(m >> 32), __builtin_amdgcn_mbcnt_lo((uint32_t)m, 0u));
}

__device__ __forceinline__ float4_t dense_chunk(const float* __restrict__ X, int64_t ld, int F, int64_t row,
                                                int tile, int j) {
  const int col = tile * kTile + j * 4;
  if (col >= F) return (float4_t)(0.f);
  float4_t v = *reinterpret_cast<const float4_t*>(X + row * ld + col);
  if (col + 1 >= F) v.y = 0.f;
  if (col + 2 >= F) v.z = 0.f;
  if (col + 3 >= F) v.w = 0.f;
  return v;
}

__device__ __forceinline__ bool nonzero(float4_t v) {
  return v.x != 0.f || v.y != 0.f || v.z != 0.f || v.w != 0.f;
}

__global__ __launch_bounds__(256) void pk_count_kernel(const float* __restrict__ X, int64_t ld, int F,
                                                       int64_t N, int tiles, int32_t* __restrict__ cnt) {
  const int lane = threadIdx.x & 63;
  const int64_t item = (int64_t)blockIdx.x * 4 + (threadIdx.x >> 6);
  if (item >= N * tiles) return;
  const int tile = (int)(item / N);
  const int64_t row = item - (int64_t)tile * N;
  const uint64_t m0 = __ballot(nonzero(dense_chunk(X, ld, F, row, tile, lane)));
  const uint64_t m1 = __ballot(nonzero(dense_chunk(X, ld, F, row, tile, 64 + lane)));
  if (lane == 0) cnt[item] = __popcll(m0) + __popcll(m1);
}

__global__ __launch_bounds__(256) void pk_fill_kernel(const float* __restrict__ X, int64_t ld, int F,
                                                      int64_t N, int tiles, const int64_t* __restrict__ ptr,
                                                      PackedHdr* __restrict__ hdr,
                                                      float4_t* __restrict__ data) {
  const int lane = threadIdx.x & 63;
  const int64_t item = (int64_t)blockIdx.x * 4 + (threadIdx.x >> 6);
  if (item >= N * tiles) return;
  const int tile = (int)(item / N);
  const int64_t row = item - (int64_t)tile * N;
  const float4_t v0 = dense_chunk(X, ld, F, row, tile, lane);
  const float4_t v1 = dense_chunk(X, ld, F, row, tile, 64 + lane);
  const uint64_t m0 = __ballot(nonzero(v0));
  const uint64_t m1 = __ballot(nonzero(v1));
  const int64_t off = ptr[item] + 1;
  if (item == 0 && lane == 0) data[0] = (float4_t)(0.f);
  if ((m0 >> lane) & 1) data[off + below(m0)] = v0;
  if ((m1 >> lane) & 1) data[off + __popcll(m0) + below(m1)] = v1;
  if (lane == 0) {
    PackedHdr h;
    h.m0 = m0;
    h.m1 = m1;
    h.off = (uint64_t)off;
    h.el = 0;
    hdr[item] = h;
  }
}

typedef unsigned int uint4_t __attribute__((ext_vector_type(4)));
constexpr uint32_t kOobOffset = 0x80000000u;

__device__ __forceinline__ uint32_t select_or_oob(uint64_t mask, uint32_t if_set, uint32_t oob) {
  uint32_t r;
  asm("v_cndmask_b32_e64 %0, %3, %1, %2" : "=v"(r) : "v"(if_set), "s"(mask), "v"(oob));
  return r;
}

template <int K>
__device__ __forceinline__ int el_phase_b_start(const int (&lim)[K], int cnt) {
  constexpr int U = 4;
  int nb = 1;
#pragma unroll
  for (int i = K - 2; i >= 0; --i)
    if (lim[i] == lim[K - 1] && nb == K - 1 - i) nb = K - i;
  if (nb != 1) return cnt;
  const int ngf = cnt / U;
  const int limA = K >= 2 ? lim[K >= 2 ? K - 2 : 0] : 0;
  const int gA = min(ngf, (limA + U - 1) / U);
  return gA < ngf ? gA * U : cnt;
}

typedef unsigned int uint2_t __attribute__((ext_vector_type(2)));

template <int K>
__device__ __forceinline__ void el_phase_b(const Job* __restrict__ jobs, int njobs, const int32_t* __restrict__ c_ids,
                                           const float* __restrict__ c_coef, const float* __restrict__ job_z,
                                           const int32_t* __restrict__ job_lim, const int32_t* __restrict__ job_order,
                                           const PackedHdr* __restrict__ hdr, const ElemEntry* __restrict__ el,
                                           uint32_t el_bytes, int64_t N, const float* __restrict__ X, int64_t ldx,
                                           int F, float* __restrict__ rows_out, float* __restrict__ prows) {
  constexpr int CH = 2;
  constexpr int U = 4;
  constexpr int W = 64;
  const int lane = threadIdx.x & 63;
  const int wid = __builtin_amdgcn_readfirstlane(blockIdx.x * kWavesPerBlock + (threadIdx.x >> 6));
  if (wid >= njobs) return;
  const int jid = __builtin_amdgcn_readfirstlane(job_order[wid]);
  const Job job = jobs[jid];
  if (job.split == 1) return;
  const int cnt = __builtin_amdgcn_readfirstlane(job.support);
  int lim[K];
#pragma unroll
  for (int i = 0; i < K; ++i) lim[i] = __builtin_amdgcn_readfirstlane(job_lim[(int64_t)jid * K + i]);
  const int j0 = el_phase_b_start<K>(lim, cnt);
  if (j0 >= cnt) return;
  float* __restrict__ rows = job.split == 2 ? prows : rows_out;
  const int col0 = blockIdx.y * kTile;
  const int Fp = F + 1;
  const int64_t rstride = (int64_t)(K + 1) * Fp;
  const int nrow = job.node_b >= 0 ? 2 : 1;
  int coff[CH];
  bool cok[CH];
#pragma unroll
  for (int c = 0; c < CH; ++c) {
    coff[c] = col0 + (lane + 64 * c) * 4;
    cok[c] = coff[c] < F;
  }
  float4_t acc[K][2][CH];
#pragma unroll
  for (int i = 0; i < K; ++i)
#pragma unroll
    for (int r = 0; r < 2; ++r)
#pragma unroll
      for (int c = 0; c < CH; ++c) acc[i][r][c] = (float4_t)(0.f);
#pragma unroll
  for (int r = 0; r < 2; ++r) {
    if (r >= nrow) break;
    const float* __restrict__ src = rows + (job.out_row + r) * rstride + (int64_t)K * Fp + 1;
#pragma unroll
    for (int c = 0; c < CH; ++c) {
      if (cok[c]) {
        const int nv = min(4, F - coff[c]);
        if (nv == 4) {
          acc[K - 1][r][c] = *reinterpret_cast<const float4_u*>(src + coff[c]);
        } else {
#pragma unroll
          for (int e = 0; e < 4; ++e)
            if (e < nv) acc[K - 1][r][c][e] = src[coff[c] + e];
        }
      }
    }
  }
  __shared__ __attribute__((aligned(16))) float2 el_lds[2 + kTile];
  float2* const eacc = el_lds + 1;
#pragma unroll
  for (int c = 0; c < CH; ++c)
#pragma unroll
    for (int e = 0; e < 4; ++e) eacc[1 + (lane + 64 * c) * 4 + e] = make_float2(acc[K - 1][0][c][e], acc[K - 1][1][c][e]);
  __syncthreads();

  const uint32_t* __restrict__ uid = reinterpret_cast<const uint32_t*>(c_ids + job.ids_off);
  const float2* __restrict__ cq = reinterpret_cast<const float2*>(c_coef) + job.coef_off + (int64_t)(K - 1) * cnt;
  const PackedHdr* __restrict__ th = hdr + (int64_t)blockIdx.y * N;
  const __amdgpu_buffer_rsrc_t ersrc =
      __builtin_amdgcn_make_buffer_rsrc(const_cast<ElemEntry*>(el), 0, (int)el_bytes, 0x00020000);
  const uint32_t oobv = kOobOffset;
  auto load_e = [&](uint32_t s, uint32_t k, uint32_t n) __attribute__((always_inline)) {
    const uint32_t a = (s + k + (uint32_t)lane) << 3;
    return __builtin_bit_cast(uint2_t, __builtin_amdgcn_raw_buffer_load_b64(
                                           ersrc, (int)(k + (uint32_t)lane < n ? a : oobv), 0, 0));
  };
  auto rmw = [&](uint2_t e, float qx, float qy) __attribute__((always_inline)) {
    float2 a = eacc[e.y];
    const float v = __builtin_bit_cast(float, e.x);
    a.x += qx * v;
    a.y += qy * v;
    eacc[e.y] = a;
  };
  struct EBuf {
    uint4_t v[U / 2];
    uint32_t s[U];
    uint32_t n[U];
  };
  const bool hi = lane >= 32;
  const uint32_t l2 = (uint32_t)(lane & 31) * 2u;
  uint32_t idn = j0 + lane < cnt ? uid[j0 + lane] : 0u;
  for (int w0 = j0; w0 < cnt; w0 += W) {
    const int nw = min(W, cnt - w0);
    const bool mine = lane < nw;
    const uint64_t rg = mine ? th[idn].el : 0ull;
    const float2 q = mine ? cq[w0 + lane] : make_float2(0.f, 0.f);
    if (w0 + W + lane < cnt) idn = uid[w0 + W + lane];
    const uint32_t es = (uint32_t)rg, en = (uint32_t)(rg >> 32);
    const int ng = (nw + U - 1) / U;
    auto issue = [&](int g, EBuf& b) __attribute__((always_inline)) {
#pragma unroll
      for (int u = 0; u < U; ++u) {
        const int j = g * U + u;
        const int l = min(j, W - 1);
        b.s[u] = (uint32_t)__builtin_amdgcn_readlane((int)es, l);
        b.n[u] = j < W ? (uint32_t)__builtin_amdgcn_readlane((int)en, l) : 0u;
      }
#pragma unroll
      for (int p = 0; p < U / 2; ++p) {
        const uint32_t sp = hi ? b.s[2 * p + 1] : b.s[2 * p];
        const uint32_t np = hi ? b.n[2 * p + 1] : b.n[2 * p];
        b.v[p] = __builtin_bit_cast(uint4_t, __builtin_amdgcn_raw_buffer_load_b128(
                                                 ersrc, (int)(l2 < np ? (sp + l2) << 3 : oobv), 0, 0));
      }
      __builtin_amdgcn_sched_barrier(0);
    };
    auto rmw_grp = [&](int g, const EBuf& b) __attribute__((always_inline)) {
#pragma unroll
      for (int p = 0; p < U / 2; ++p) {
        const auto ev = __builtin_amdgcn_permlane32_swap(b.v[p].x, b.v[p].z, false, false);
        const auto sl = __builtin_amdgcn_permlane32_swap(b.v[p].y, b.v[p].w, false, false);
#pragma unroll
        for (int r = 0; r < 2; ++r) {
          const int u = 2 * p + r;
          const int l = min(g * U + u, W - 1);
          const float qx = __builtin_bit_cast(float, __builtin_amdgcn_readlane(__builtin_bit_cast(int, q.x), l));
          const float qy = __builtin_bit_cast(float, __builtin_amdgcn_readlane(__builtin_bit_cast(int, q.y), l));
          uint2_t e;
          e.x = ev[r];
          e.y = sl[r];
          rmw(e, qx, qy);
          if (__builtin_expect(b.n[u] > 64, 0)) {
#pragma nounroll
            for (uint32_t k = 64; k < b.n[u]; k += 64)
              rmw(load_e(b.s[u], k, b.n[u]), qx, qy);
          }
        }
      }
      __builtin_amdgcn_sched_barrier(0);
    };
    EBuf bA, bB;
    issue(0, bA);
    for (int g = 0; g < ng; g += 2) {
      issue(g + 1, bB);
      rmw_grp(g, bA);
      if (g + 1 < ng) {
        issue(g + 2, bA);
        rmw_grp(g + 1, bB);
      }
    }
  }
  __syncthreads();
#pragma unroll
  for (int c = 0; c < CH; ++c)
#pragma unroll
    for (int e = 0; e < 4; ++e) {
      const float2 a = eacc[1 + (lane + 64 * c) * 4 + e];
      acc[K - 1][0][c][e] = a.x;
      acc[K - 1][1][c][e] = a.y;
    }
  write_pair_rows_part<K, CH, K - 1, K, false, true>(job, jid, acc, coff, cok, job_z, X, ldx, F, rows,
                                                     blockIdx.y == 0);
}

template <int K, int MINNB, int EL>
constexpr int packed_min_waves() {
  return EL == 3 ? 8 : (K <= 3 || (MINNB == 2 && K <= 5)) ? 4 : 1;
}

template <int K, int MINNB, int EL>
__global__ __launch_bounds__(kWavesPerBlock * 64)
__attribute__((amdgpu_waves_per_eu(packed_min_waves<K, MINNB, EL>()))) void gather_packed_kernel(
    const Job* __restrict__ jobs, int njobs, const int32_t* __restrict__ c_ids,
    const float* __restrict__ c_coef, const float* __restrict__ job_z,
    const int32_t* __restrict__ job_lim, const int32_t* __restrict__ job_order,
    const PackedHdr* __restrict__ hdr,
    const float4_t* __restrict__ data, uint32_t data_bytes, const ElemEntry* __restrict__ el, uint32_t el_bytes,
    int64_t N, const float* __restrict__ X, int64_t ldx, int F, float* __restrict__ rows_out,
    float* __restrict__ prows) {
  if constexpr (EL == 3) {
    el_phase_b<K>(jobs, njobs, c_ids, c_coef, job_z, job_lim, job_order, hdr, el, el_bytes, N, X, ldx, F, rows_out,
                  prows);
    return;
  }
  constexpr int CH = 2;
  constexpr int U = 4;
  const int lane = threadIdx.x & 63;
  const int wid = __builtin_amdgcn_readfirstlane(blockIdx.x * kWavesPerBlock + (threadIdx.x >> 6));
  if (wid >= njobs) return;
  const int jid = __builtin_amdgcn_readfirstlane(job_order[wid]);
  const int col0 = blockIdx.y * kTile;
  const Job job = jobs[jid];
  if (job.split == 1) return;
  float* __restrict__ rows = job.split == 2 ? prows : rows_out;
  const int cnt = __builtin_amdgcn_readfirstlane(job.support);
  const uint32_t* __restrict__ uid = reinterpret_cast<const uint32_t*>(c_ids + job.ids_off);
  const float2* __restrict__ cf = reinterpret_cast<const float2*>(c_coef) + job.coef_off;
  const PackedHdr* __restrict__ th = hdr + (int64_t)blockIdx.y * N;
  const __amdgpu_buffer_rsrc_t rsrc =
      __builtin_amdgcn_make_buffer_rsrc(const_cast<float4_t*>(data), 0, (int)data_bytes, 0x00020000);
  const uint32_t oobv = kOobOffset;
  int lim[K];
#pragma unroll
  for (int i = 0; i < K; ++i) lim[i] = __builtin_amdgcn_readfirstlane(job_lim[(int64_t)jid * K + i]);

  int coff[CH];
  bool cok[CH];
#pragma unroll
  for (int c = 0; c < CH; ++c) {
    coff[c] = col0 + (lane + 64 * c) * 4;
    cok[c] = coff[c] < F;
  }
  float4_t acc[K][2][CH];
#pragma unroll
  for (int i = 0; i < K; ++i)
#pragma unroll
    for (int r = 0; r < 2; ++r)
#pragma unroll
      for (int c = 0; c < CH; ++c) acc[i][r][c] = (float4_t)(0.f);

  auto hdr_of = [&](uint32_t id) __attribute__((always_inline)) -> PackedHdr {
    static_assert(sizeof(PackedHdr) == 32, "the shift below");
    return *reinterpret_cast<const PackedHdr*>(reinterpret_cast<const char*>(th) + (id << 5));
  };
  auto load_hdrs = [&](int g, PackedHdr(&h)[U]) __attribute__((always_inline)) {
    uint32_t id[U];
#pragma unroll
    for (int u = 0; u < U; ++u) id[u] = uid[g * U + u];
    __builtin_amdgcn_sched_barrier(0);
#pragma unroll
    for (int u = 0; u < U; ++u) h[u] = hdr_of(id[u]);
    __builtin_amdgcn_sched_barrier(0);
  };
  auto load_ids = [&](int g, uint32_t(&id)[U]) __attribute__((always_inline)) {
#pragma unroll
    for (int u = 0; u < U; ++u) id[u] = uid[g * U + u];
    __builtin_amdgcn_sched_barrier(0);
  };
  auto hdrs_from = [&](const uint32_t(&id)[U], PackedHdr(&h)[U]) __attribute__((always_inline)) {
#pragma unroll
    for (int u = 0; u < U; ++u) h[u] = hdr_of(id[u]);
    __builtin_amdgcn_sched_barrier(0);
  };
  auto hdrs_from_late = [&](const uint32_t(&id)[U], PackedHdr(&h)[U]) __attribute__((always_inline)) {
    uint32_t idv[U];
#pragma unroll
    for (int u = 0; u < U; ++u) idv[u] = id[u];
    asm volatile("" : "+s"(idv[0]), "+s"(idv[1]), "+s"(idv[2]), "+s"(idv[3]));
    static_assert(U == 4, "the opaque statement above lists four ids");
#pragma unroll
    for (int u = 0; u < U; ++u) h[u] = hdr_of(idv[u]);
    __builtin_amdgcn_sched_barrier(0);
  };
  auto issue = [&](const PackedHdr(&h)[U], float4_t(&v)[U][CH], bool valid = true) __attribute__((always_inline)) {
#pragma unroll
    for (int u = 0; u < U; ++u) {
      const uint32_t base = valid ? (uint32_t)h[u].off : (kOobOffset >> 4);
      const uint32_t a0 = (base + (uint32_t)below(h[u].m0)) << 4;
      const uint32_t a1 = (base + (uint32_t)__popcll(h[u].m0) + (uint32_t)below(h[u].m1)) << 4;
      v[u][0] = __builtin_bit_cast(float4_t, __builtin_amdgcn_raw_buffer_load_b128(
                                                 rsrc, (int)select_or_oob(h[u].m0, a0, oobv), 0, 0));
      v[u][1] = __builtin_bit_cast(float4_t, __builtin_amdgcn_raw_buffer_load_b128(
                                                 rsrc, (int)select_or_oob(h[u].m1, a1, oobv), 0, 0));
    }
    __builtin_amdgcn_sched_barrier(0);
  };
  auto fma_from = [&](auto first, auto last, int g, const float4_t(&v)[U][CH]) __attribute__((always_inline)) {
    constexpr int I0 = decltype(first)::value, I1 = decltype(last)::value;
#pragma unroll
    for (int i = I0; i < I1; ++i) {
#pragma unroll
      for (int u = 0; u < U; ++u) {
        const float2 q = cf[(int64_t)i * cnt + g * U + u];
#pragma unroll
        for (int c = 0; c < CH; ++c) {
          acc[i][0][c] += q.x * v[u][c];
          acc[i][1][c] += q.y * v[u][c];
        }
      }
    }
  };
  auto tail_rows = [&](auto first, auto last, int j0) __attribute__((always_inline)) {
    constexpr int I0 = decltype(first)::value, I1 = decltype(last)::value;
    for (int j = j0; j < cnt; ++j) {
      const PackedHdr h = hdr_of(uid[j]);
      const uint32_t base = (uint32_t)h.off;
      const uint32_t a0 = (base + (uint32_t)below(h.m0)) << 4;
      const uint32_t a1 = (base + (uint32_t)__popcll(h.m0) + (uint32_t)below(h.m1)) << 4;
      float4_t v[CH];
      v[0] = __builtin_bit_cast(float4_t, __builtin_amdgcn_raw_buffer_load_b128(
                                              rsrc, (int)select_or_oob(h.m0, a0, oobv), 0, 0));
      v[1] = __builtin_bit_cast(float4_t, __builtin_amdgcn_raw_buffer_load_b128(
                                              rsrc, (int)select_or_oob(h.m1, a1, oobv), 0, 0));
#pragma unroll
      for (int i = I0; i < I1; ++i) {
        const float2 q = cf[(int64_t)i * cnt + j];
#pragma unroll
        for (int c = 0; c < CH; ++c) {
          acc[i][0][c] += q.x * v[c];
          acc[i][1][c] += q.y * v[c];
        }
      }
    }
  };

  __shared__ __attribute__((aligned(16))) float2 el_lds[EL == 1 || EL == 2 ? 2 + kTile : kStageDwords / 2];
  static_assert(2 * (2 + kTile) >= kStageDwords, "the staging records share the element accumulators' LDS");
  uint32_t* const stage = reinterpret_cast<uint32_t*>(el_lds);
  auto pass2 = [&](auto first, auto last, int g0, int g1) __attribute__((always_inline)) {
    constexpr int I0 = decltype(first)::value;
    constexpr int NO_RAW = decltype(last)::value - I0;
    constexpr int NO = NO_RAW > 0 ? NO_RAW : 1;
    if (NO_RAW <= 0) return;
    if (g1 <= g0) return;
    int g = g0;
    if constexpr (NO <= 3) {
      static_assert(4 + 2 * U * 3 <= kRecStride && kRecStride <= 64, "a record is one dword per lane");
      constexpr int WG = kPrefixWindow / U;
      PackedHdr h[U];
      float4_t vA[U][CH], vB[U][CH];
      uint32_t rec;
      const int rlast = g1 * U - 1;
      auto fill = [&](int gw) __attribute__((always_inline)) {
        const int r0 = gw * U;
        const uint32_t oq = (uint32_t)min(lane, rlast - r0);
        const uint32_t oi = (uint32_t)min(lane + 2 * U, rlast - r0);
        const uint32_t idv = (uid + r0)[oi];
        float2 qv[NO];
#pragma unroll
        for (int i = 0; i < NO; ++i) qv[i] = (cf + ((int64_t)(I0 + i) * cnt + r0))[oq];
        __syncthreads();
        int ll = lane;
        asm volatile("" : "+v"(ll));
        uint32_t* const r = stage + (ll >> 2) * kRecStride;
        r[ll & 3] = idv;
#pragma unroll
        for (int i = 0; i < NO; ++i)
          *reinterpret_cast<uint2_t*>(r + 4 + (i * U + (ll & 3)) * 2) =
              uint2_t{__builtin_bit_cast(uint32_t, qv[i].x), __builtin_bit_cast(uint32_t, qv[i].y)};
        __syncthreads();
        rec = stage[lane];
        __builtin_amdgcn_sched_barrier(0);
      };
      auto ids_at = [&](uint32_t r, int l0, uint32_t(&id)[U]) __attribute__((always_inline)) {
#pragma unroll
        for (int u = 0; u < U; ++u) id[u] = (uint32_t)__builtin_amdgcn_readlane((int)r, l0 + u);
      };
      auto q_of = [&](float2(&qa)[NO][U]) __attribute__((always_inline)) {
#pragma unroll
        for (int i = 0; i < NO; ++i)
#pragma unroll
          for (int u = 0; u < U; ++u) {
            qa[i][u].x = __builtin_bit_cast(float, __builtin_amdgcn_readlane((int)rec, 4 + (i * U + u) * 2));
            qa[i][u].y = __builtin_bit_cast(float, __builtin_amdgcn_readlane((int)rec, 5 + (i * U + u) * 2));
          }
      };
      auto fma_rec = [&](const float2(&qa)[NO][U], const float4_t(&v)[U][CH]) __attribute__((always_inline)) {
#pragma unroll
        for (int u = 0; u < U; ++u) {
#pragma unroll
          for (int i = 0; i < NO; ++i)
#pragma unroll
            for (int c = 0; c < CH; ++c) {
              acc[I0 + i][0][c] += qa[i][u].x * v[u][c];
              acc[I0 + i][1][c] += qa[i][u].y * v[u][c];
            }
          __builtin_amdgcn_sched_barrier(0);
        }
      };
      auto half = [&](int snext, float4_t(&vi)[U][CH], bool valid, const float4_t(&vf)[U][CH]) __attribute__((always_inline)) {
        issue(h, vi, valid);
        uint32_t id[U];
        float2 qa[NO][U];
        ids_at(rec, 0, id);
        q_of(qa);
        __builtin_amdgcn_sched_barrier(0);
        hdrs_from(id, h);
        rec = stage[snext * kRecStride + lane];
        __builtin_amdgcn_sched_barrier(0);
        fma_rec(qa, vf);
      };
      {
        const uint32_t id0v = (uid + g0 * U)[(uint32_t)min(lane, min(2 * U - 1, rlast - g0 * U))];
        fill(g0);
        uint32_t id[U];
        ids_at(id0v, 0, id);
        hdrs_from(id, h);
        issue(h, vA);
        ids_at(id0v, U, id);
        hdrs_from(id, h);
      }
      int s = 0;
      for (; g + 1 < g1; g += 2) {
        if (s == WG) {
          fill(g);
          s = 0;
        }
        half(s + 1, vB, true, vA);
        half(s + 2, vA, g + 2 < g1, vB);
        s += 2;
      }
      if (g < g1) {
        if (s == WG) fill(g);
        float2 qa[NO][U];
        q_of(qa);
        __builtin_amdgcn_sched_barrier(0);
        fma_rec(qa, vA);
      }
    } else {
      PackedHdr hA[U], hB[U];
      float4_t vA[U][CH], vB[U][CH];
      uint32_t idn[U];
      load_hdrs(g0, hA);
      issue(hA, vA);
      if (g1 - g0 > 1) load_hdrs(g0 + 1, hB);
      if (g1 - g0 > 2) load_ids(g0 + 2, idn);
      auto fma_g = [&](int gq, const float4_t(&v)[U][CH]) {
        fma_from(first, last, gq, v);
        __builtin_amdgcn_sched_barrier(0);
      };
      for (; g + 4 < g1; g += 2) {
        issue(hB, vB);
        hdrs_from(idn, hA);
        load_ids(g + 3, idn);
        fma_g(g, vA);
        issue(hA, vA);
        hdrs_from(idn, hB);
        load_ids(g + 4, idn);
        fma_g(g + 1, vB);
      }
      fma_g(g, vA);
      ++g;
      for (; g < g1; ++g) {
        load_hdrs(g, hA);
        issue(hA, vA);
        fma_g(g, vA);
      }
    }
  };

  auto pass3 = [&](int g0, int g1) __attribute__((always_inline)) {
    const int nB = g1 - g0;
    if (nB <= 0) return;
    auto grp = [&](int k) { return g0 + min(k, nB - 1); };
    uint32_t idX[U], idY[U];
    PackedHdr hX[U], hY[U];
    float2 qX[U], qY[U];
    float4_t v0[U][CH], v1[U][CH], v2[U][CH];
    auto load_q = [&](int g, float2(&q)[U]) {
#pragma unroll
      for (int u = 0; u < U; ++u) q[u] = cf[(int64_t)(K - 1) * cnt + g * U + u];
      __builtin_amdgcn_sched_barrier(0);
    };
    auto fma_q = [&](const float2(&q)[U], const float4_t(&v)[U][CH]) {
#pragma unroll
      for (int u = 0; u < U; ++u) {
#pragma unroll
        for (int c = 0; c < CH; ++c) {
          acc[K - 1][0][c] += q[u].x * v[u][c];
          acc[K - 1][1][c] += q[u].y * v[u][c];
        }
      }
      __builtin_amdgcn_sched_barrier(0);
    };
    load_ids(grp(0), idX);
    hdrs_from(idX, hX);
    issue(hX, v0);
    load_ids(grp(1), idX);
    hdrs_from(idX, hY);
    issue(hY, v1, 1 < nB);
    load_ids(grp(2), idX);
    hdrs_from(idX, hX);
    load_ids(grp(3), idX);
    load_q(grp(0), qX);
#define S3GRL_GATHER_STEP(k, IDr, IDl, Hr, Hl, Qr, Ql, Vissue, Vfma) \
  hdrs_from_late(IDr, Hl);                                            \
  load_ids(grp((k) + 4), IDl);                                        \
  load_q(grp((k) + 1), Ql);                                           \
  issue(Hr, Vissue, (k) + 2 < nB);                                    \
  fma_q(Qr, Vfma);
    for (int k = 0; k < nB; k += 6) {
      S3GRL_GATHER_STEP(k, idX, idY, hX, hY, qX, qY, v2, v0)
      S3GRL_GATHER_STEP(k + 1, idY, idX, hY, hX, qY, qX, v0, v1)
      S3GRL_GATHER_STEP(k + 2, idX, idY, hX, hY, qX, qY, v1, v2)
      S3GRL_GATHER_STEP(k + 3, idY, idX, hY, hX, qY, qX, v2, v0)
      S3GRL_GATHER_STEP(k + 4, idX, idY, hX, hY, qX, qY, v0, v1)
      S3GRL_GATHER_STEP(k + 5, idY, idX, hY, hX, qY, qX, v1, v2)
    }
#undef S3GRL_GATHER_STEP
// ... 367 lines not shown
```

### s3grl_amd/csrc/s3grl_structure.hip

```cpp

#include <cstdlib>

#include "s3grl_internal.hpp"
#include "s3grl_device.hpp"
#include "s3grl_link_classes.hpp"

namespace s3grl {
namespace {

constexpr int kCountList = 1024;

template <int G, int kCountBlock, bool EXT = false>
__global__ __launch_bounds__(kCountBlock) void count_kernel(
    const int32_t* __restrict__ indptr, const int32_t* __restrict__ indices, int N, int W,
    const int64_t* __restrict__ links, int hops, int plus, int K, int hubs,
    const WalkSets ws, const int32_t* __restrict__ partner, const int32_t* __restrict__ mirror_of,
    int32_t* __restrict__ n_nodes, int32_t* __restrict__ p_nodes, int32_t* __restrict__ n_rows,
    int32_t* __restrict__ n_jobs, int32_t* __restrict__ lvl_max, int32_t* __restrict__ err_flag,
    unsigned long long* __restrict__ tot_nodes_alg, HopSampling smp, int32_t* __restrict__ stash,
    int slot, int32_t* __restrict__ lvl_stash, const int32_t* __restrict__ cn_indptr,
    const int32_t* __restrict__ cn_indices, int full_p, uint32_t* __restrict__ ext, int64_t ext_stride,
    int link_base, const int32_t* __restrict__ perm) {
  extern __shared__ uint32_t smem[];
  const bool walks = walks_on(ws);
// ... 906 lines not shown
                               int64_t npieces, Job* gjobs, int32_t* g_lim, int32_t* g_order, int32_t* piece_job) {
  if (njobs == 0) return S3GRL_OK;
  hipLaunchKernelGGL(split_fill_kernel, dim3((unsigned)((njobs + 255) / 256)), dim3(256), 0, ctx->stream, jobs,
                     job_lim, job_order, njobs, K, seg_shift, piece_off, npieces, gjobs, g_lim, g_order, piece_job);
  S3GRL_HIP_TRY(hipGetLastError());
  return S3GRL_OK;
}

s3grl_status launch_combine(s3grl_context* ctx, const s3grl_plan* p, const float* prows, const float* X,
                            int64_t ldx, int64_t F, float* rows) {
  if (p->njobs == 0 || p->npieces == 0) return S3GRL_OK;
  hipLaunchKernelGGL(combine_kernel, dim3((unsigned)p->npieces, 2), dim3(256), 0, ctx->stream, p->jobs,
                     p->piece_off, p->piece_job, p->job_z, p->cfg.sign_k, prows, X, ldx, (int)F, rows);
  S3GRL_HIP_TRY(hipGetLastError());
  return S3GRL_OK;
}

s3grl_status launch_mirror_rows(s3grl_context* ctx, const int32_t* partner, int64_t L,
                                int32_t* n_rows) {
  if (L == 0) return S3GRL_OK;
  hipLaunchKernelGGL(mirror_rows_kernel, dim3((unsigned)((L + 255) / 256)), dim3(256), 0, ctx->stream,
                     partner, L, n_rows);
  S3GRL_HIP_TRY(hipGetLastError());
  return S3GRL_OK;
}

s3grl_status launch_count(s3grl_context* ctx, const s3grl_graph* g, const int64_t* links, int64_t L,
                          int hops, int plus, int K, WalkSets ws,
                          const int32_t* partner, const int32_t* mirror_of, int32_t* n_nodes, int32_t* p_nodes,
                          int32_t* n_rows, int32_t* n_jobs, int32_t* lvl_max, int32_t* err_flag,
                          int64_t* tot_nodes_alg, HopSampling smp, int32_t* stash, int slot,
                          int32_t* lvl_stash, const int32_t* perm) {
  if (L == 0) return S3GRL_OK;
  const int W = words_for(g->num_nodes);
  const int nbm = (hops <= 1 || walks_on(ws)) ? 2 : 3;
  const int nsets = nbm + (hop_sampling_on(smp) ? 1 : 0);
  const size_t lds = (size_t)(nsets * W + 8 + kHubWords + kCountList) * 4;
  const bool sparse = (double)g->nnz / (double)std::max<int64_t>(g->num_nodes, 1) <= 6.0;
  const int32_t* cn_ip = g->directed ? g->out_indptr : g->indptr;
  const int32_t* cn_ix = g->directed ? g->out_indices : g->indices;
  if (lds > 163840 || getenv("S3GRL_FORCE_EXT_BITMAPS")) {
    const int64_t stride = ((int64_t)nsets * W + 63) / 64 * 64;
    const int chunk = (int)std::min<int64_t>(L, std::max<int64_t>(256, ((int64_t)1 << 29) / (stride * 4)));
    Transient tmp{ctx, {}};
    void* q = nullptr;
    S3GRL_TRY(ctx->arena.alloc((size_t)stride * 4 * chunk, &q));
    tmp.ptrs.push_back(q);
    const size_t lds_ext = (size_t)(8 + kHubWords + kCountList) * 4;
    auto kern = sparse ? count_kernel<4, 256, true> : count_kernel<8, 256, true>;
    for (int64_t base = 0; base < L; base += chunk) {
      const int64_t cnt = std::min<int64_t>(chunk, L - base);
      hipLaunchKernelGGL(kern, dim3((unsigned)cnt), dim3(256), lds_ext, ctx->stream, g->indptr, g->indices,
                         (int)g->num_nodes, W, links, hops, plus, K, g->max_degree > kHubArmDegree ? 1 : 0, ws,
                         partner, mirror_of, n_nodes, p_nodes, n_rows, n_jobs, lvl_max, err_flag,
                         reinterpret_cast<unsigned long long*>(tot_nodes_alg), smp, stash, slot, lvl_stash, cn_ip,
                         cn_ix, g->directed ? 1 : 0, static_cast<uint32_t*>(q), stride, (int)base, perm);
      S3GRL_HIP_TRY(hipGetLastError());
    }
    S3GRL_HIP_TRY(hipStreamSynchronize(ctx->stream));
    return S3GRL_OK;
  }
  const bool small = lds <= 24 * 1024;
  auto kern = small ? (sparse ? count_kernel<4, 128> : count_kernel<8, 128>)
                    : (sparse ? count_kernel<4, 256> : count_kernel<8, 256>);
  S3GRL_HIP_TRY(hipFuncSetAttribute(reinterpret_cast<const void*>(kern),
                                    hipFuncAttributeMaxDynamicSharedMemorySize, (int)lds));
  hipLaunchKernelGGL(kern, dim3((unsigned)L), dim3(small ? 128 : 256), lds, ctx->stream, g->indptr,
                     g->indices, (int)g->num_nodes, W, links, hops, plus, K,
                     g->max_degree > kHubArmDegree ? 1 : 0, ws, partner, mirror_of, n_nodes,
                     p_nodes, n_rows, n_jobs, lvl_max, err_flag,
                     reinterpret_cast<unsigned long long*>(tot_nodes_alg), smp, stash, slot, lvl_stash,
                     cn_ip, cn_ix, g->directed ? 1 : 0, nullptr, 0, 0, perm);
  S3GRL_HIP_TRY(hipGetLastError());
  return S3GRL_OK;
}

constexpr int kOrderBuckets = 256;
constexpr int kOrderShift = 5;

__device__ __forceinline__ int order_bucket(int n) {
  return kOrderBuckets - 1 - min(n >> kOrderShift, kOrderBuckets - 1);
}

constexpr int kOrderThreads = 1024;

__global__ __launch_bounds__(kOrderThreads) void order_hist_kernel(
    const int32_t* __restrict__ n_nodes, const int32_t* __restrict__ n_jobs, int64_t L, int64_t per_block,
    int32_t* __restrict__ hist) {
  __shared__ int h[kOrderBuckets];
  const int t = threadIdx.x;
  if (t < kOrderBuckets) h[t] = 0;
  __syncthreads();
  const int64_t l0 = (int64_t)blockIdx.x * per_block, l1 = min(l0 + per_block, L);
  for (int64_t l = l0 + t; l < l1; l += kOrderThreads) {
    const int nj = n_jobs[l];
    if (nj > 0) atomicAdd(&h[order_bucket(n_nodes[l])], nj);
  }
  __syncthreads();
  if (t < kOrderBuckets && h[t]) atomicAdd(&hist[t], h[t]);
}

__global__ void order_scan_kernel(int32_t* __restrict__ hist ) {
  __shared__ int sh[kOrderBuckets];
  const int t = threadIdx.x;
  sh[t] = hist[t];
  __syncthreads();
  if (t == 0) {
    int run = 0;
    for (int b = 0; b < kOrderBuckets; ++b) {
      const int c = sh[b];
      sh[b] = run;
      run += c;
    }
  }
  __syncthreads();
  hist[t] = sh[t];
}

__global__ __launch_bounds__(kOrderThreads) void order_fill_kernel(
    const int32_t* __restrict__ n_nodes, const int32_t* __restrict__ n_jobs,
    const int64_t* __restrict__ job_off, int64_t L, int64_t per_block, int32_t* __restrict__ cursor,
    int32_t* __restrict__ job_order) {
  __shared__ int h[kOrderBuckets];
  __shared__ int base[kOrderBuckets];
  const int t = threadIdx.x;
  if (t < kOrderBuckets) h[t] = 0;
  __syncthreads();
  const int64_t l0 = (int64_t)blockIdx.x * per_block, l1 = min(l0 + per_block, L);
  for (int64_t l = l0 + t; l < l1; l += kOrderThreads) {
    const int nj = n_jobs[l];
    if (nj > 0) atomicAdd(&h[order_bucket(n_nodes[l])], nj);
  }
  __syncthreads();
  if (t < kOrderBuckets) {
    base[t] = h[t] ? atomicAdd(&cursor[t], h[t]) : 0;
    h[t] = 0;
  }
  __syncthreads();
  for (int64_t l = l0 + t; l < l1; l += kOrderThreads) {
    const int nj = n_jobs[l];
    if (nj <= 0) continue;
    const int b = order_bucket(n_nodes[l]);
    const int at = base[b] + atomicAdd(&h[b], nj);
    const int j0 = (int)job_off[l];
    for (int j = 0; j < nj; ++j) job_order[at + j] = j0 + j;
  }
}

__global__ void perm_jobs_kernel(const int32_t* __restrict__ perm, const int32_t* __restrict__ n_jobs, int64_t L,
                                 int32_t* __restrict__ cnt) {
  const int64_t i = (int64_t)blockIdx.x * blockDim.x + threadIdx.x;
  if (i < L) cnt[i] = n_jobs[perm[i]];
}

__global__ void perm_fill_kernel(const int32_t* __restrict__ perm, const int32_t* __restrict__ n_jobs,
                                 const int64_t* __restrict__ job_off, const int64_t* __restrict__ at, int64_t L,
                                 int32_t* __restrict__ job_order) {
  const int64_t i = (int64_t)blockIdx.x * blockDim.x + threadIdx.x;
  if (i >= L) return;
  const int l = perm[i];
  const int nj = n_jobs[l];
  const int j0 = (int)job_off[l];
  const int64_t a = at[i];
  for (int j = 0; j < nj; ++j) job_order[a + j] = j0 + j;
}

s3grl_status launch_job_order(s3grl_context* ctx, const int32_t* n_nodes, const int32_t* n_jobs,
                              const int64_t* job_off, int64_t L, int32_t* hist ,
                              int32_t* job_order, const int32_t* perm, int32_t* scratch_cnt,
                              int64_t* scratch_off, int64_t* scan_ws) {
  if (L == 0) return S3GRL_OK;
  if (perm) {
    const unsigned grid = (unsigned)((L + 255) / 256);
    hipLaunchKernelGGL(perm_jobs_kernel, dim3(grid), dim3(256), 0, ctx->stream, perm, n_jobs, L, scratch_cnt);
    S3GRL_HIP_TRY(hipGetLastError());
    S3GRL_TRY(launch_scan_i32_to_i64(ctx, scratch_cnt, L, scratch_off, scan_ws));
    hipLaunchKernelGGL(perm_fill_kernel, dim3(grid), dim3(256), 0, ctx->stream, perm, n_jobs, job_off, scratch_off,
                       L, job_order);
    S3GRL_HIP_TRY(hipGetLastError());
    return S3GRL_OK;
  }
  S3GRL_HIP_TRY(hipMemsetAsync(hist, 0, kOrderBuckets * sizeof(int32_t), ctx->stream));
  const int64_t per_block = std::max<int64_t>((L + 255) / 256, 4 * kOrderThreads);
  const unsigned grid = (unsigned)((L + per_block - 1) / per_block);
  hipLaunchKernelGGL(order_hist_kernel, dim3(grid), dim3(kOrderThreads), 0, ctx->stream, n_nodes, n_jobs, L,
                     per_block, hist);
  hipLaunchKernelGGL(order_scan_kernel, dim3(1), dim3(kOrderBuckets), 0, ctx->stream, hist);
  hipLaunchKernelGGL(order_fill_kernel, dim3(grid), dim3(kOrderThreads), 0, ctx->stream, n_nodes, n_jobs, job_off,
                     L, per_block, hist, job_order);
  S3GRL_HIP_TRY(hipGetLastError());
  return S3GRL_OK;
}

int64_t scan_workspace_elems(int64_t n) { return (n + kScanTile - 1) / kScanTile + 1; }

s3grl_status launch_scan3(s3grl_context* ctx, const int32_t* in0, const int32_t* in1, const int32_t* in2,
                          int64_t n, int64_t* out0, int64_t* out1, int64_t* out2, int64_t* workspace3,
                          int64_t* max0, int64_t* max1, int64_t* totals) {
  const int64_t nb = (n + kScanTile - 1) / kScanTile;
  const int64_t wsz = scan_workspace_elems(n);
  Scan3 a;
  a.in[0] = in0; a.in[1] = in1; a.in[2] = in2;
  a.out[0] = out0; a.out[1] = out1; a.out[2] = out2;
  for (int y = 0; y < 3; ++y) {
    a.part[y] = workspace3 + y * wsz;
    a.total_out[y] = totals ? totals + y : nullptr;
  }
  a.max_out[0] = reinterpret_cast<long long*>(max0);
  a.max_out[1] = reinterpret_cast<long long*>(max1);
  a.max_out[2] = nullptr;
  hipLaunchKernelGGL(scan3_partials_kernel, dim3((unsigned)nb, 3), dim3(256), 0, ctx->stream, a, n);
  hipLaunchKernelGGL(scan3_top_kernel, dim3(3), dim3(1024), 0, ctx->stream, a, nb, n);
  hipLaunchKernelGGL(scan3_apply_kernel, dim3((unsigned)nb, 3), dim3(256), 0, ctx->stream, a, n);
  S3GRL_HIP_TRY(hipGetLastError());
  return S3GRL_OK;
}

s3grl_status launch_scan_i32_to_i64(s3grl_context* ctx, const int32_t* in, int64_t n, int64_t* out,
                                    int64_t* workspace) {
  if (n == 0) {
    S3GRL_HIP_TRY(hipMemsetAsync(out, 0, 8, ctx->stream));
    return S3GRL_OK;
  }
  const int64_t nb = (n + kScanTile - 1) / kScanTile;
  hipLaunchKernelGGL(scan_partials_kernel, dim3((unsigned)nb), dim3(256), 0, ctx->stream, in, n,
                     workspace);
  hipLaunchKernelGGL(scan_top_kernel, dim3(1), dim3(1024), 0, ctx->stream, workspace, nb, out + n);
  hipLaunchKernelGGL(scan_apply_kernel, dim3((unsigned)nb), dim3(256), 0, ctx->stream, in, n,
                     workspace, out);
  S3GRL_HIP_TRY(hipGetLastError());
  return S3GRL_OK;
}


bool sparse_mode_for(const s3grl_graph* g) {
  if (getenv("S3GRL_FORCE_HASH")) return true;
  return 3 * (size_t)words_for(g->num_nodes) * 4 > 24 * 1024;
}

int num_class_lists() { return kNumListsAll; }

bool onehop_mode_for(const s3grl_graph* g) {
  if (getenv("S3GRL_FORCE_ONEHOP")) return true;
  return sparse_mode_for(g);
}

s3grl_status build_forward_rows(s3grl_context* ctx, s3grl_graph* g) {
  const int64_t N = g->num_nodes;
  Transient tmp{ctx, {}};
  void* q = nullptr;
  S3GRL_TRY(ctx->arena.alloc((size_t)N * 4, &q));
  tmp.ptrs.push_back(q);
  int32_t* cnt = static_cast<int32_t*>(q);
  S3GRL_TRY(ctx->arena.alloc((size_t)(N + 1) * 8, &q));
  tmp.ptrs.push_back(q);
  int64_t* off64 = static_cast<int64_t*>(q);
  S3GRL_TRY(ctx->arena.alloc((size_t)scan_workspace_elems(N) * 8, &q));
  tmp.ptrs.push_back(q);
  int64_t* ws = static_cast<int64_t*>(q);
  const unsigned grid = (unsigned)((N + 255) / 256);
  hipLaunchKernelGGL(fwd_count_kernel, dim3(grid), dim3(256), 0, ctx->stream, g->indptr, g->indices, N, cnt);
  S3GRL_HIP_TRY(hipGetLastError());
  S3GRL_TRY(launch_scan_i32_to_i64(ctx, cnt, N, off64, ws));
  S3GRL_HIP_TRY(hipMemcpyAsync(ctx->h_scalars, off64 + N, 8, hipMemcpyDeviceToHost, ctx->stream));
  S3GRL_HIP_TRY(hipStreamSynchronize(ctx->stream));
  const int64_t fnnz = ctx->h_scalars[0];
  S3GRL_TRY(ctx->arena.alloc((size_t)(N + 1) * 4, &q));
  g->fwd_indptr = static_cast<int32_t*>(q);
  S3GRL_TRY(ctx->arena.alloc((size_t)std::max<int64_t>(fnnz, 1) * 4, &q));
  g->fwd_indices = static_cast<int32_t*>(q);
  S3GRL_TRY(ctx->arena.alloc((size_t)N * 2, &q));
  g->fwd_deg = static_cast<uint16_t*>(q);
  hipLaunchKernelGGL(fwd_fill_kernel, dim3((unsigned)((N + 1 + 255) / 256)), dim3(256), 0, ctx->stream,
                     g->indptr, g->indices, N, off64, g->fwd_indptr, g->fwd_indices, g->fwd_deg);
  S3GRL_HIP_TRY(hipGetLastError());
  S3GRL_HIP_TRY(hipStreamSynchronize(ctx->stream));
  return S3GRL_OK;
}

s3grl_status launch_count1(s3grl_context* ctx, const s3grl_graph* g, const int64_t* links, int64_t L,
                           int plus, int K, const int32_t* partner, const int32_t* mirror_of,
                           int32_t* n_nodes, int32_t* p_nodes, int32_t* n_rows, int32_t* n_jobs,
                           int32_t* lvl_max, int32_t* e_cap, int32_t* err_flag, int64_t* tot_nodes_alg,
                           int64_t* tot_oriented, const int32_t* perm, int64_t* x_cap) {
  if (L == 0) return S3GRL_OK;
  hipLaunchKernelGGL(count1_kernel, dim3((unsigned)((L + kCount1Waves - 1) / kCount1Waves)),
                     dim3(64 * kCount1Waves), 0, ctx->stream, g->indptr, g->indices, g->fwd_deg,
                     (int)g->num_nodes, links, L, plus, K, partner, mirror_of, n_nodes, p_nodes, n_rows,
                     n_jobs, lvl_max, e_cap, err_flag, reinterpret_cast<unsigned long long*>(tot_nodes_alg),
                     reinterpret_cast<unsigned long long*>(tot_oriented), perm, g->hub,
                     (x_cap && g->hub.nh > 0) ? x_cap : nullptr);
  S3GRL_HIP_TRY(hipGetLastError());
  return S3GRL_OK;
}

s3grl_status launch_classify(s3grl_context* ctx, const s3grl_graph* g, int cn_cap, int K,
                             const int32_t* n_nodes, const int32_t* p_nodes,
                             const int32_t* lvl_max, int64_t L, int32_t* class_count,
                             int32_t* class_list, bool allow_hash, const int32_t* e_cap, int stash_slot,
                             const int32_t* perm, const int64_t* x_cap, const int32_t* csr_e, bool tiny_ok) {
  if (L == 0) return S3GRL_OK;
  const char* segs = getenv("S3GRL_SPLIT_SEG_SHIFT");
  const int tiny_max_n = (tiny_ok && !getenv("S3GRL_NO_TINY") && !(segs && atoi(segs) < 6)) ? kTinyNodes : 0;
  ClassBounds cb = class_bounds(g->num_nodes, cn_cap, K);
  const bool dm = allow_hash && stash_slot > 0 && dm_mode_for(g);
  if (cb.b[kNumClasses - 1] < 0 || getenv("S3GRL_FORCE_EXT_BITMAPS")) {
    for (int c = 0; c < kNumClasses; ++c) cb.b[c] = -1;
  }
  ClassBounds hb{};
  static_assert(kHubClasses <= kNumClasses, "hub class bounds travel in a ClassBounds");
  static_assert(kHubClasses < kNumClasses, "one more entry for the test hook");
  for (int c = 0; c < kHubClasses; ++c) hb.b[c] = hub_class_bound(c, cn_cap, K);
  hb.b[kHubClasses] = getenv("S3GRL_FORCE_HUB_SLICES") ? 1 : 0;
  CsrBounds csrb{};
  for (int c = 0; c < kCsrClasses; ++c) csrb.b[c] = csr_class_bound(c, cn_cap, K);
  hipLaunchKernelGGL(classify_kernel, dim3((unsigned)((L + 255) / 256)), dim3(256), 0, ctx->stream,
                     n_nodes, p_nodes, lvl_max, L, cb, dm ? 2 : ((allow_hash && sparse_mode_for(g)) ? 1 : 0),
                     dm ? class_bounds_dm(g->num_nodes, cn_cap, K) : class_bounds_sparse(cn_cap, K), e_cap,
                     class_bounds_full(cn_cap, K),
                     getenv("S3GRL_FORCE_BM_HBM") ? 0 : (1 << 30),
                     dm ? std::min(stash_slot + 2, 65535) : 0, dm ? dm_class_mask_for(g, cn_cap, K) : 0,
                     class_count, class_list, perm, x_cap, hb, csr_e, csrb, words_for(g->num_nodes), tiny_max_n);
  S3GRL_HIP_TRY(hipGetLastError());
  return S3GRL_OK;
}


s3grl_status launch_links(s3grl_context* ctx, const s3grl_graph* g, const int64_t* links, int64_t L,
                          const int32_t* class_list, const int32_t* class_count_host, int hops,
                          int plus, int cn_cap, int full_stats, int K, WalkSets ws, const int32_t* p_nodes,
                          const LinkOut& out, HopSampling smp, const int32_t* stash, int slot,
                          const int32_t* e_cap, const int32_t* new_of_old, const int64_t* x_cap,
                          const uint16_t* csr_cnt, const int32_t* csr_e, int sop2) {
  if (L == 0) return S3GRL_OK;
  Transient scratch_owner{ctx, {}};
  char* scratch = nullptr;
  int64_t scratch_stride = 0;
  int bm_ext_words = 0, gs_chunk = 0;
  if (class_count_host[kNumClasses] > 0) {
    scratch_stride = ((int64_t)class_count_host[kNumClasses + 1] + 255) / 256 * 256;
    int64_t slices = class_count_host[kNumClasses];
    if (4 * (int64_t)link_fixed_words(g->num_nodes, cn_cap, K) > 163840 || getenv("S3GRL_FORCE_EXT_BITMAPS")) {
      bm_ext_words = (3 * words_for(g->num_nodes) + 63) / 64 * 64;
      scratch_stride += (int64_t)bm_ext_words * 4;
      gs_chunk = (int)std::min<int64_t>(slices, std::max<int64_t>(64, ((int64_t)1 << 29) / scratch_stride));
      slices = gs_chunk;
    }
    void* q = nullptr;
    S3GRL_TRY(ctx->arena.alloc((size_t)scratch_stride * slices, &q));
    scratch_owner.ptrs.push_back(q);
    scratch = static_cast<char*>(q);
  }
  LinkArgs a{g, links, class_list, hops, plus, cn_cap, full_stats, ws, p_nodes, out, scratch, scratch_stride,
             getenv("S3GRL_DEBUG_STAMPS") ? reinterpret_cast<unsigned long long*>(ctx->d_scalars + 16) : nullptr,
             smp, stash, slot, e_cap, nullptr, 0, 0, 0, new_of_old,
             (out.old_of_new && !getenv("S3GRL_NO_LEAF_WALK")) ? g->deg_le2_from : -1,
             DirGraph{g->out_indptr, g->out_indices, g->in_indptr, g->in_indices}, bm_ext_words, gs_chunk, 0,
             x_cap, nullptr, 0, 0, csr_cnt, csr_e, sop2};
  if (class_count_host[kHubBase + kHubClasses] > 0) {
    const int64_t xmax = ((int64_t)class_count_host[29] + 63) / 64 * 64;
    a.hub_slice_words = 2 * xmax;
    a.hub_slice_grid = (int)std::min<int64_t>(class_count_host[kHubBase + kHubClasses], 256);
    void* q = nullptr;
    S3GRL_TRY(ctx->arena.alloc((size_t)a.hub_slice_words * 4 * a.hub_slice_grid, &q));
    scratch_owner.ptrs.push_back(q);
    a.hub_slices = static_cast<uint32_t*>(q);
  }
  if (class_count_host[kFullBig] > 0) {
    a.bm_stride_words = ((int64_t)class_count_host[31] / 2 + 2 + (class_count_host[31] + 2) / 2 + 63) / 64 * 64;
    a.big_need = 163840 - 4 * full_fixed_words(cn_cap, K);
    a.bm_grid = (int)std::min<int64_t>(class_count_host[kFullBig], 256);
    void* q = nullptr;
    S3GRL_TRY(ctx->arena.alloc((size_t)a.bm_stride_words * 4 * a.bm_grid, &q));
    scratch_owner.ptrs.push_back(q);
    a.bm_scratch = static_cast<uint32_t*>(q);
  }
  switch (K) {
    case 1: return launch_links_k<1>(ctx, a, L, class_count_host);
    case 2: return launch_links_k<2>(ctx, a, L, class_count_host);
    case 3: return launch_links_k<3>(ctx, a, L, class_count_host);
    case 4: return launch_links_k<4>(ctx, a, L, class_count_host);
    case 5: return launch_links_k<5>(ctx, a, L, class_count_host);
    case 6: return launch_links_k<6>(ctx, a, L, class_count_host);
    case 7: return launch_links_k<7>(ctx, a, L, class_count_host);
    case 8: return launch_links_k<8>(ctx, a, L, class_count_host);
    default:
      set_last_error("sign_k must be in 1..8");
      return S3GRL_ERR_INVALID_ARGUMENT;
  }
}


s3grl_status launch_dists(s3grl_context* ctx, const int64_t* node_off, const int32_t* lvl, int64_t L,
                          int8_t* dists) {
  if (L == 0) return S3GRL_OK;
  hipLaunchKernelGGL(dists_kernel, dim3((unsigned)L), dim3(256), 0, ctx->stream, node_off, lvl, L,
                     dists);
  S3GRL_HIP_TRY(hipGetLastError());
  return S3GRL_OK;
}

}

S3GRL_DEFINE_TOUCH(structure)
```

Before: 17.46 million link pairs/s.

## Stop zero-filling coefficient tails and mask them in gathers; align LDS class bounds

The link kernels now zero only the first few coefficient entries past each hop's limit, instead of zeroing the full support range. The gather kernels (dense, narrow and sparse) load per-job hop limits and mask coefficients beyond them in registers, which keeps the results correct. Separately, the LDS class bounds are snapped to residency granules, and the hub words are counted only when the graph has hubs, so more blocks may fit per CU. In exchange, the gathers do an extra limit load and a select per coefficient.

```diff
diff --git a/s3grl_amd/csrc/s3grl_api.hip b/s3grl_amd/csrc/s3grl_api.hip
--- a/s3grl_amd/csrc/s3grl_api.hip
+++ b/s3grl_amd/csrc/s3grl_api.hip
@@ -1057,7 +1057,8 @@
   auto gather = [&](const GatherView& v) -> s3grl_status {
     if (f->sparse) return launch_gather_sparse(ctx, p, v, f, rows);
     if (f->packed) return launch_gather_packed(ctx, p, v, f, rows);
-    return launch_gather(ctx, v, p->c_ids, p->c_coef, p->cfg.sign_k, f->dense, f->ld, f->F, rows, p->hub_order);
+    return launch_gather(ctx, v, p->c_ids, p->c_coef, p->cfg.sign_k, f->dense, f->ld, f->F, rows, p->hub_order,
+                         (p->walk_plan ? 1 : p->cfg.num_hops) >= 2);
   };
   if (p->npieces == 0) {
     S3GRL_TRY(gather(GatherView{p->jobs, p->njobs, p->job_z, p->job_lim, p->job_order, nullptr}));
diff --git a/s3grl_amd/csrc/s3grl_csr.hip b/s3grl_amd/csrc/s3grl_csr.hip
--- a/s3grl_amd/csrc/s3grl_csr.hip
+++ b/s3grl_amd/csrc/s3grl_csr.hip
@@ -232,6 +232,7 @@
     pair_rows(pr, R, pos_src, pos_dst, cnpos, pos_a, pos_b);
     const int row_hop = pr == 0 ? 0 : 1;
     const int support = lvl_end[min(K + row_hop, nlev - 1)];
+    const int zero_end = coef_zero_end(lvl_end[min(K - 1 + row_hop, nlev - 1)], support);
     for (int w = tid; w < n; w += T) {
       cur[w] = make_float2(0.f, 0.f);
       nxs[w] = make_float2(0.f, 0.f);
@@ -283,7 +284,7 @@
         }
       }
       if (!last)
-        for (int t = limit + tid; t < support; t += T) coef[cidx(i, t)] = make_float2(0.f, 0.f);
+        for (int t = limit + tid; t < zero_end; t += T) coef[cidx(i, t)] = make_float2(0.f, 0.f);
       __syncthreads();
       float2* tmp = s_in;
       s_in = s_out;
diff --git a/s3grl_amd/csrc/s3grl_features.hip b/s3grl_amd/csrc/s3grl_features.hip
--- a/s3grl_amd/csrc/s3grl_features.hip
+++ b/s3grl_amd/csrc/s3grl_features.hip
@@ -4,6 +4,7 @@
 
 #include "s3grl_internal.hpp"
 #include "s3grl_device.hpp"
+#include "s3grl_gather_common.hpp"
 
 namespace s3grl {
 namespace {
@@ -130,7 +131,7 @@
 template <int K>
 __global__ __launch_bounds__(256) void gather_sparse_kernel(
     const Job* __restrict__ jobs, int njobs, const int32_t* __restrict__ c_ids,
-    const float* __restrict__ c_coef, const float* __restrict__ job_z,
+    const float* __restrict__ c_coef, const float* __restrict__ job_z, const int32_t* __restrict__ job_lim,
     const int64_t* __restrict__ xptr, const Entry* __restrict__ ent, const float* __restrict__ X,
     int64_t ldx, int64_t N, int F, float* __restrict__ rows_out, float* __restrict__ prows) {
   extern __shared__ float2 lds2[];
@@ -149,6 +150,12 @@
   const int32_t* __restrict__ ids = c_ids + job.ids_off;
   const float2* __restrict__ cf = reinterpret_cast<const float2*>(c_coef) + job.coef_off;
   const int64_t* __restrict__ xp = xptr + (int64_t)tile * N;
+  int lim[K];
+  load_limits<K>(job_lim, jid, lim);
+  auto coef = [&](int i, int j) __attribute__((always_inline)) -> float2 {
+    const float2 q = cf[(int64_t)i * cnt + j];
+    return i == K - 1 ? q : coef_or_zero(q, j, lim[i]);
+  };
 
   {
     float4* a4 = reinterpret_cast<float4*>(acc);
@@ -176,7 +183,7 @@
     for (int u = 0; u < U; ++u) {
       float2 q[K];
 #pragma unroll
-      for (int i = 0; i < K; ++i) q[i] = cf[(int64_t)i * cnt + j + u];
+      for (int i = 0; i < K; ++i) q[i] = coef(i, j + u);
       if (beg[u] + lane < end[u]) scatter_entry<K>(acc, e[u].col, e[u].val, q);
       for (int64_t p = beg[u] + 64 + lane; p - lane < end[u]; p += 64) {
         if (p < end[u]) {
@@ -191,7 +198,7 @@
     const int64_t b = xp[id], en = xp[id + 1];
     float2 q[K];
 #pragma unroll
-    for (int i = 0; i < K; ++i) q[i] = cf[(int64_t)i * cnt + j];
+    for (int i = 0; i < K; ++i) q[i] = coef(i, j);
     for (int64_t p = b + lane; p - lane < en; p += 64) {
       if (p < en) {
         const Entry t = ent[p];
@@ -237,7 +244,7 @@
   S3GRL_HIP_TRY(hipFuncSetAttribute(reinterpret_cast<const void*>(kern),
                                     hipFuncAttributeMaxDynamicSharedMemorySize, (int)lds));
   hipLaunchKernelGGL(kern, dim3(gx, (unsigned)f->tiles), dim3(256), lds, ctx->stream, v.jobs,
-                     (int)v.njobs, p->c_ids, p->c_coef, v.job_z, f->sp_ptr,
+                     (int)v.njobs, p->c_ids, p->c_coef, v.job_z, v.job_lim, f->sp_ptr,
                      reinterpret_cast<const Entry*>(f->sp_ent), f->dense, f->ld, f->N, (int)f->F, rows, v.prows);
   S3GRL_HIP_TRY(hipGetLastError());
   return S3GRL_OK;
diff --git a/s3grl_amd/csrc/s3grl_gather.hip b/s3grl_amd/csrc/s3grl_gather.hip
--- a/s3grl_amd/csrc/s3grl_gather.hip
+++ b/s3grl_amd/csrc/s3grl_gather.hip
@@ -10,12 +10,12 @@
 constexpr int kUnroll = 8;
 constexpr int kNarrowUnroll = 8;
 
-template <int K, int CH>
+template <int K, int CH, bool LIM>
 __global__ __launch_bounds__(kWavesPerBlock * 64) void gather_kernel(
     const Job* __restrict__ jobs, int njobs, const int32_t* __restrict__ c_ids,
     const float* __restrict__ c_coef, const float* __restrict__ job_z, const float* __restrict__ X,
     int64_t ldx, int F, float* __restrict__ rows_out, float* __restrict__ prows,
-    const int32_t* __restrict__ job_order) {
+    const int32_t* __restrict__ job_order, const int32_t* __restrict__ job_lim) {
   const int lane = threadIdx.x & 63;
   const int wid = __builtin_amdgcn_readfirstlane(blockIdx.x * kWavesPerBlock + (threadIdx.x >> 6));
   if (wid >= njobs) return;
@@ -27,6 +27,13 @@
   const int cnt = __builtin_amdgcn_readfirstlane(job.support);
   const int32_t* __restrict__ ids = c_ids + job.ids_off;
   const float2* __restrict__ cf = reinterpret_cast<const float2*>(c_coef) + job.coef_off;
+  int lim[K];
+  if constexpr (LIM) load_limits<K>(job_lim, jid, lim);
+  auto coef = [&](int i, int j) __attribute__((always_inline)) -> float2 {
+    const float2 q = cf[(int64_t)i * cnt + j];
+    if constexpr (!LIM) return q;
+    return i == K - 1 ? q : coef_or_zero(q, j, lim[i]);
+  };
 
   int coff[CH];
   bool cok[CH];
@@ -61,7 +68,7 @@
     for (int i = 0; i < K; ++i) {
 #pragma unroll
       for (int u = 0; u < kUnroll; ++u) {
-        const float2 q = cf[(int64_t)i * cnt + j + u];
+        const float2 q = coef(i, j + u);
 #pragma unroll
         for (int c = 0; c < CH; ++c) {
           acc[i][0][c] += q.x * v[u][c];
@@ -77,7 +84,7 @@
       const float4_t v = cok[c] ? *reinterpret_cast<const float4_t*>(xr + coff[c]) : (float4_t)(0.f);
 #pragma unroll
       for (int i = 0; i < K; ++i) {
-        const float2 q = cf[(int64_t)i * cnt + j];
+        const float2 q = coef(i, j);
         acc[i][0][c] += q.x * v;
         acc[i][1][c] += q.y * v;
       }
@@ -90,12 +97,12 @@
 typedef float float2_t __attribute__((ext_vector_type(2)));
 typedef float float2_u __attribute__((ext_vector_type(2), aligned(4)));
 
-template <int K>
+template <int K, bool LIM>
 __global__ __launch_bounds__(kWavesPerBlock * 64) void gather_narrow_kernel(
     const Job* __restrict__ jobs, int njobs, const int32_t* __restrict__ c_ids,
     const float* __restrict__ c_coef, const float* __restrict__ job_z, const float* __restrict__ X,
     int64_t ldx, int F, float* __restrict__ rows_out, float* __restrict__ prows,
-    const int32_t* __restrict__ job_order) {
+    const int32_t* __restrict__ job_order, const int32_t* __restrict__ job_lim) {
   constexpr int U = K <= 3 ? kNarrowUnroll : (K == 4 ? 6 : (K == 5 ? 5 : (K == 6 ? 4 : 3)));
   const int lane = threadIdx.x & 63;
   const int wid = __builtin_amdgcn_readfirstlane(blockIdx.x * kWavesPerBlock + (threadIdx.x >> 6));
@@ -107,6 +114,13 @@
   const int cnt = __builtin_amdgcn_readfirstlane(job.support);
   const int32_t* __restrict__ ids = c_ids + job.ids_off;
   const float2* __restrict__ cf = reinterpret_cast<const float2*>(c_coef) + job.coef_off;
+  int lim[K];
+  if constexpr (LIM) load_limits<K>(job_lim, jid, lim);
+  auto coef = [&](int i, int j) __attribute__((always_inline)) -> float2 {
+    const float2 q = cf[(int64_t)i * cnt + j];
+    if constexpr (!LIM) return q;
+    return i == K - 1 ? q : coef_or_zero(q, j, lim[i]);
+  };
   const int coff = lane * 2;
   const bool col_ok = coff < F;
   const uint32_t voff = (uint32_t)(col_ok ? coff : 0) * 4u;
@@ -143,7 +157,7 @@
 #pragma unroll
       for (int i = 0; i < K; ++i)
 #pragma unroll
-        for (int u = 0; u < U; ++u) q[i][u] = cf[(int64_t)i * cnt + g * U + u];
+        for (int u = 0; u < U; ++u) q[i][u] = coef(i, g * U + u);
       __builtin_amdgcn_sched_barrier(0);
 #pragma unroll
       for (int i = 0; i < K; ++i) {
@@ -160,7 +174,7 @@
     const float2_t v = row_of(ids[j]);
 #pragma unroll
     for (int i = 0; i < K; ++i) {
-      const float2 q = cf[(int64_t)i * cnt + j];
+      const float2 q = coef(i, j);
       acc[i][0] += q.x * v;
       acc[i][1] += q.y * v;
     }
@@ -197,46 +211,51 @@
   }
 }
 
-template <int K>
+template <int K, bool LIM>
 s3grl_status launch_k(s3grl_context* ctx, const Job* jobs, int64_t njobs, const int32_t* c_ids,
                       const float* c_coef, const float* job_z, const float* X, int64_t ldx,
-                      int64_t F, float* rows, float* prows, const int32_t* job_order) {
+                      int64_t F, float* rows, float* prows, const int32_t* job_order, const int32_t* job_lim) {
   hipStream_t stream = ctx->stream;
   const unsigned gx = (unsigned)((njobs + kWavesPerBlock - 1) / kWavesPerBlock);
   if (F <= 128 && ldx < ((int64_t)1 << 30)) {
-    hipLaunchKernelGGL((gather_narrow_kernel<K>), dim3(gx, 1), dim3(kWavesPerBlock * 64), 0, stream,
-                       jobs, (int)njobs, c_ids, c_coef, job_z, X, ldx, (int)F, rows, prows, job_order);
+    hipLaunchKernelGGL((gather_narrow_kernel<K, LIM>), dim3(gx, 1), dim3(kWavesPerBlock * 64), 0, stream,
+                       jobs, (int)njobs, c_ids, c_coef, job_z, X, ldx, (int)F, rows, prows, job_order, job_lim);
   } else if (F <= 256) {
-    hipLaunchKernelGGL((gather_kernel<K, 1>), dim3(gx, 1), dim3(kWavesPerBlock * 64), 0, stream,
-                       jobs, (int)njobs, c_ids, c_coef, job_z, X, ldx, (int)F, rows, prows, job_order);
+    hipLaunchKernelGGL((gather_kernel<K, 1, LIM>), dim3(gx, 1), dim3(kWavesPerBlock * 64), 0, stream,
+                       jobs, (int)njobs, c_ids, c_coef, job_z, X, ldx, (int)F, rows, prows, job_order, job_lim);
   } else {
     const unsigned gy = (unsigned)((F + 511) / 512);
-    hipLaunchKernelGGL((gather_kernel<K, 2>), dim3(gx, gy), dim3(kWavesPerBlock * 64), 0,
-                       stream, jobs, (int)njobs, c_ids, c_coef, job_z, X, ldx, (int)F, rows, prows, job_order);
+    hipLaunchKernelGGL((gather_kernel<K, 2, LIM>), dim3(gx, gy), dim3(kWavesPerBlock * 64), 0,
+                       stream, jobs, (int)njobs, c_ids, c_coef, job_z, X, ldx, (int)F, rows, prows, job_order, job_lim);
   }
   S3GRL_HIP_TRY(hipGetLastError());
   return S3GRL_OK;
 }
 
+template <int K>
+s3grl_status launch_k(s3grl_context* ctx, const GatherView& v, const int32_t* c_ids, const float* c_coef,
+                      const float* X, int64_t ldx, int64_t F, float* rows, const int32_t* order, bool limits) {
+  if (K >= 2 && limits)
+    return launch_k<K, (K >= 2)>(ctx, v.jobs, v.njobs, c_ids, c_coef, v.job_z, X, ldx, F, rows, v.prows, order, v.job_lim);
+  return launch_k<K, false>(ctx, v.jobs, v.njobs, c_ids, c_coef, v.job_z, X, ldx, F, rows, v.prows, order, v.job_lim);
+}
+
 }
 
 s3grl_status launch_gather(s3grl_context* ctx, const GatherView& v, const int32_t* c_ids,
                            const float* c_coef, int K, const float* X, int64_t ldx, int64_t F, float* rows,
-                           bool in_job_order) {
-  const Job* jobs = v.jobs;
-  const int64_t njobs = v.njobs;
-  const float* job_z = v.job_z;
+                           bool in_job_order, bool limits) {
   const int32_t* order = in_job_order ? v.job_order : nullptr;
-  if (njobs == 0) return S3GRL_OK;
+  if (v.njobs == 0) return S3GRL_OK;
   switch (K) {
-    case 1: return launch_k<1>(ctx, jobs, njobs, c_ids, c_coef, job_z, X, ldx, F, rows, v.prows, order);
-    case 2: return launch_k<2>(ctx, jobs, njobs, c_ids, c_coef, job_z, X, ldx, F, rows, v.prows, order);
-    case 3: return launch_k<3>(ctx, jobs, njobs, c_ids, c_coef, job_z, X, ldx, F, rows, v.prows, order);
-    case 4: return launch_k<4>(ctx, jobs, njobs, c_ids, c_coef, job_z, X, ldx, F, rows, v.prows, order);
-    case 5: return launch_k<5>(ctx, jobs, njobs, c_ids, c_coef, job_z, X, ldx, F, rows, v.prows, order);
-    case 6: return launch_k<6>(ctx, jobs, njobs, c_ids, c_coef, job_z, X, ldx, F, rows, v.prows, order);
-    case 7: return launch_k<7>(ctx, jobs, njobs, c_ids, c_coef, job_z, X, ldx, F, rows, v.prows, order);
-    case 8: return launch_k<8>(ctx, jobs, njobs, c_ids, c_coef, job_z, X, ldx, F, rows, v.prows, order);
+    case 1: return launch_k<1>(ctx, v, c_ids, c_coef, X, ldx, F, rows, order, limits);
+    case 2: return launch_k<2>(ctx, v, c_ids, c_coef, X, ldx, F, rows, order, limits);
+    case 3: return launch_k<3>(ctx, v, c_ids, c_coef, X, ldx, F, rows, order, limits);
+    case 4: return launch_k<4>(ctx, v, c_ids, c_coef, X, ldx, F, rows, order, limits);
+    case 5: return launch_k<5>(ctx, v, c_ids, c_coef, X, ldx, F, rows, order, limits);
+    case 6: return launch_k<6>(ctx, v, c_ids, c_coef, X, ldx, F, rows, order, limits);
+    case 7: return launch_k<7>(ctx, v, c_ids, c_coef, X, ldx, F, rows, order, limits);
+    case 8: return launch_k<8>(ctx, v, c_ids, c_coef, X, ldx, F, rows, order, limits);
     default:
       set_last_error("sign_k must be in 1..8");
       return S3GRL_ERR_INVALID_ARGUMENT;
diff --git a/s3grl_amd/csrc/s3grl_gather_common.hpp b/s3grl_amd/csrc/s3grl_gather_common.hpp
--- a/s3grl_amd/csrc/s3grl_gather_common.hpp
+++ b/s3grl_amd/csrc/s3grl_gather_common.hpp
@@ -7,6 +7,15 @@
 
 typedef float float4_t __attribute__((ext_vector_type(4)));
 typedef float float4_u __attribute__((ext_vector_type(4), aligned(4)));
+
+__device__ __forceinline__ float2 coef_or_zero(float2 q, int j, int lim) {
+  return j < lim ? q : make_float2(0.f, 0.f);
+}
+template <int K>
+__device__ __forceinline__ void load_limits(const int32_t* __restrict__ job_lim, int jid, int (&lim)[K]) {
+#pragma unroll
+  for (int i = 0; i < K; ++i) lim[i] = __builtin_amdgcn_readfirstlane(job_lim[(int64_t)jid * K + i]);
+}
 
 template <int K, int CH, int I0, int I1, bool XROW, bool ZCOL>
 __device__ __forceinline__ void write_pair_rows_part(const Job& job, int jid, const float4_t (&acc)[K][2][CH],
diff --git a/s3grl_amd/csrc/s3grl_internal.hpp b/s3grl_amd/csrc/s3grl_internal.hpp
--- a/s3grl_amd/csrc/s3grl_internal.hpp
+++ b/s3grl_amd/csrc/s3grl_internal.hpp
@@ -82,6 +82,11 @@
   const int s0 = (t >> seg_shift) << seg_shift;
   const int len = min(1 << seg_shift, support - s0);
   return piece_coef_off(s0, K) + (int64_t)i * len + (t - s0);
+}
+
+constexpr int kCoefGroup = 4;
+__host__ __device__ __forceinline__ int coef_zero_end(int lim_middle, int support) {
+  return lim_middle + kCoefGroup - 1 < support ? lim_middle + kCoefGroup - 1 : support;
 }
 
 struct LinkOut {
@@ -498,7 +503,7 @@
                           int8_t* dists);
 s3grl_status launch_gather(s3grl_context* ctx, const GatherView& v, const int32_t* c_ids,
                            const float* c_coef, int K, const float* X, int64_t ldx, int64_t F, float* rows,
-                           bool in_job_order = false);
+                           bool in_job_order, bool limits );
 s3grl_status build_packed_rows(s3grl_context* ctx, s3grl_features* f, double max_density, bool elements);
 s3grl_status build_element_rows(s3grl_context* ctx, s3grl_features* f);
 s3grl_status launch_gather_packed(s3grl_context* ctx, const s3grl_plan* p, const GatherView& v,
diff --git a/s3grl_amd/csrc/s3grl_link_classes.hpp b/s3grl_amd/csrc/s3grl_link_classes.hpp
--- a/s3grl_amd/csrc/s3grl_link_classes.hpp
+++ b/s3grl_amd/csrc/s3grl_link_classes.hpp
@@ -18,6 +18,10 @@
   int C = 64;
   while (C < 2 * n) C <<= 1;
   return 8 * C + link_lds_need(n, p) + link_bm_bytes(n, p);
+}
+
+__host__ __device__ __forceinline__ int link_tail_words(int cn_cap, int K, bool hubs) {
+  return cn_cap + kMaxLevels + 4 * K + 32 + (hubs ? kHubWords : 0);
 }
 
 struct ClassBounds {
@@ -59,27 +63,49 @@
 
 static inline int words_for(int64_t N) { return (int)((N + 31) / 32); }
 
-static inline int link_fixed_words(int64_t num_nodes, int cn_cap, int K) {
-  return 3 * words_for(num_nodes) + cn_cap + kMaxLevels + 4 * K + 32 + kHubWords;
+static inline bool hub_armed(const s3grl_graph* g) { return g->max_degree > kHubArmDegree; }
+
+static inline int link_fixed_words(const s3grl_graph* g, int cn_cap, int K) {
+  return 3 * words_for(g->num_nodes) + link_tail_words(cn_cap, K, hub_armed(g));
 }
-static inline int link_fixed_words_sparse(int cn_cap, int K) {
-  return cn_cap + kMaxLevels + 4 * K + 32 + kHubWords;
+static inline int link_fixed_words_sparse(const s3grl_graph* g, int cn_cap, int K) {
+  return link_tail_words(cn_cap, K, hub_armed(g));
+}
+static inline int link_fixed_words_dm(const s3grl_graph* g, int cn_cap, int K) {
+  return 16 * words_for(g->num_nodes) + link_tail_words(cn_cap, K, hub_armed(g));
 }
 
 static constexpr int kNominalBounds[kNumClasses] = {6144, 12288, 24576, 49152, 98304, 163840};
 
-static ClassBounds class_bounds(int64_t num_nodes, int cn_cap, int K) {
-  const int* nominal = kNominalBounds;
-  int avail = 163840 - 4 * link_fixed_words(num_nodes, cn_cap, K);
-  if (const char* e = getenv("S3GRL_LDS_BUDGET")) avail = std::min(avail, atoi(e));
+constexpr int kLdsBytes = 163840;
+constexpr int kLdsGranule = 1280;
+static inline int lds_share(int k) { return kLdsBytes / k / kLdsGranule * kLdsGranule; }
+
+static ClassBounds cut_bounds(int fixed_bytes, int avail) {
   ClassBounds cb;
-  for (int c = 0; c < kNumClasses; ++c) cb.b[c] = std::min(nominal[c], avail);
+  for (int c = 0; c < kNumClasses; ++c) {
+    const int k0 = std::max(1, kLdsBytes / std::max(fixed_bytes + kNominalBounds[c], 1));
+    const int lo = lds_share(k0 + 1) - fixed_bytes, hi = lds_share(k0) - fixed_bytes;
+    int b = kNominalBounds[c];
+    if (hi > 0) b = (lo > 0 && kNominalBounds[c] - lo < hi - kNominalBounds[c]) ? lo : hi;
+    cb.b[c] = std::min(b, avail);
+  }
   cb.b[kNumClasses - 1] = avail;
   return cb;
 }
-static ClassBounds class_bounds_sparse(int cn_cap, int K) {
+static inline int lds_resident(size_t lds) {
+  return (int)(kLdsBytes / std::max<size_t>((lds + kLdsGranule - 1) / kLdsGranule * kLdsGranule, kLdsGranule));
+}
+
+static ClassBounds class_bounds(const s3grl_graph* g, int cn_cap, int K) {
+  const int fixed = 4 * link_fixed_words(g, cn_cap, K);
+  int avail = kLdsBytes - fixed;
+  if (const char* e = getenv("S3GRL_LDS_BUDGET")) avail = std::min(avail, atoi(e));
+  return cut_bounds(fixed, avail);
+}
+static ClassBounds class_bounds_sparse(const s3grl_graph* g, int cn_cap, int K) {
   static const int nominal[kNumClasses] = {4096, 8192, 16384, 32768, 65536, 131072};
-  const int avail = 163840 - 4 * link_fixed_words_sparse(cn_cap, K);
+  const int avail = kLdsBytes - 4 * link_fixed_words_sparse(g, cn_cap, K);
   ClassBounds cb;
   for (int c = 0; c < kNumClasses; ++c) cb.b[c] = std::min(nominal[c], avail);
   return cb;
@@ -99,16 +125,9 @@
   return lds <= 40 * 1024 ? 256 : (lds <= 80 * 1024 ? 512 : 1024);
 }
 
-static inline int link_fixed_words_dm(int64_t num_nodes, int cn_cap, int K) {
-  return 16 * words_for(num_nodes) + cn_cap + kMaxLevels + 4 * K + 32 + kHubWords;
-}
-static ClassBounds class_bounds_dm(int64_t num_nodes, int cn_cap, int K) {
-  const int* nominal = kNominalBounds;
-  const int avail = 163840 - 4 * link_fixed_words_dm(num_nodes, cn_cap, K);
-  ClassBounds cb;
-  for (int c = 0; c < kNumClasses; ++c) cb.b[c] = std::min(nominal[c], avail);
-  cb.b[kNumClasses - 1] = avail;
-  return cb;
+static ClassBounds class_bounds_dm(const s3grl_graph* g, int cn_cap, int K) {
+  const int fixed = 4 * link_fixed_words_dm(g, cn_cap, K);
+  return cut_bounds(fixed, kLdsBytes - fixed);
 }
 
 static bool dm_mode_for(const s3grl_graph* g) {
@@ -117,19 +136,18 @@
 }
 
 static int waves_per_cu(size_t lds, int c) {
-  return std::min<int>(32, (int)(163840 / std::max<size_t>(lds, 1)) * (threads_for_class(lds, c) / 64));
+  return std::min<int>(32, lds_resident(lds) * (threads_for_class(lds, c) / 64));
 }
 static int dm_class_mask_for(const s3grl_graph* g, int cn_cap, int K) {
-  const ClassBounds bb = class_bounds(g->num_nodes, cn_cap, K), bd = class_bounds_dm(g->num_nodes, cn_cap, K);
+  const ClassBounds bb = class_bounds(g, cn_cap, K), bd = class_bounds_dm(g, cn_cap, K);
   int mask = 0;
   for (int c = 0; c < kNumClasses; ++c) {
     if (bd.b[c] <= 0) continue;
     if (bb.b[c] <= 0) { mask |= 1 << c; continue; }
-    const int wb = waves_per_cu((size_t)4 * link_fixed_words(g->num_nodes, cn_cap, K) + bb.b[c], c);
-    const int wd = waves_per_cu((size_t)4 * link_fixed_words_dm(g->num_nodes, cn_cap, K) + bd.b[c], c);
-    const size_t lb = (size_t)4 * link_fixed_words(g->num_nodes, cn_cap, K) + bb.b[c];
-    const size_t ld = (size_t)4 * link_fixed_words_dm(g->num_nodes, cn_cap, K) + bd.b[c];
-    if (c == 0 && 2 * std::min<size_t>(163840 / ld, 16) < std::min<size_t>(163840 / lb, 16)) continue;
+    const size_t lb = (size_t)4 * link_fixed_words(g, cn_cap, K) + bb.b[c];
+    const size_t ld = (size_t)4 * link_fixed_words_dm(g, cn_cap, K) + bd.b[c];
+    const int wb = waves_per_cu(lb, c), wd = waves_per_cu(ld, c);
+    if (c == 0 && 2 * std::min(lds_resident(ld), 16) < std::min(lds_resident(lb), 16)) continue;
     if (5 * wd >= 4 * wb) mask |= 1 << c;
   }
   return mask;
diff --git a/s3grl_amd/csrc/s3grl_packed.hip b/s3grl_amd/csrc/s3grl_packed.hip
--- a/s3grl_amd/csrc/s3grl_packed.hip
+++ b/s3grl_amd/csrc/s3grl_packed.hip
@@ -286,6 +286,7 @@
   }
   constexpr int CH = 2;
   constexpr int U = 4;
+  static_assert(U == kCoefGroup, "the link kernels' zero fill covers phase A's last group");
   const int lane = threadIdx.x & 63;
   const int wid = __builtin_amdgcn_readfirstlane(blockIdx.x * kWavesPerBlock + (threadIdx.x >> 6));
   if (wid >= njobs) return;
diff --git a/s3grl_amd/csrc/s3grl_structure.hip b/s3grl_amd/csrc/s3grl_structure.hip
--- a/s3grl_amd/csrc/s3grl_structure.hip
+++ b/s3grl_amd/csrc/s3grl_structure.hip
@@ -1232,7 +1232,7 @@
   if (L == 0) return S3GRL_OK;
   const char* segs = getenv("S3GRL_SPLIT_SEG_SHIFT");
   const int tiny_max_n = (tiny_ok && !getenv("S3GRL_NO_TINY") && !(segs && atoi(segs) < 6)) ? kTinyNodes : 0;
-  ClassBounds cb = class_bounds(g->num_nodes, cn_cap, K);
+  ClassBounds cb = class_bounds(g, cn_cap, K);
   const bool dm = allow_hash && stash_slot > 0 && dm_mode_for(g);
   if (cb.b[kNumClasses - 1] < 0 || getenv("S3GRL_FORCE_EXT_BITMAPS")) {
     for (int c = 0; c < kNumClasses; ++c) cb.b[c] = -1;
@@ -1246,7 +1246,7 @@
   for (int c = 0; c < kCsrClasses; ++c) csrb.b[c] = csr_class_bound(c, cn_cap, K);
   hipLaunchKernelGGL(classify_kernel, dim3((unsigned)((L + 255) / 256)), dim3(256), 0, ctx->stream,
                      n_nodes, p_nodes, lvl_max, L, cb, dm ? 2 : ((allow_hash && sparse_mode_for(g)) ? 1 : 0),
-                     dm ? class_bounds_dm(g->num_nodes, cn_cap, K) : class_bounds_sparse(cn_cap, K), e_cap,
+                     dm ? class_bounds_dm(g, cn_cap, K) : class_bounds_sparse(g, cn_cap, K), e_cap,
                      class_bounds_full(cn_cap, K),
                      getenv("S3GRL_FORCE_BM_HBM") ? 0 : (1 << 30),
                      dm ? std::min(stash_slot + 2, 65535) : 0, dm ? dm_class_mask_for(g, cn_cap, K) : 0,
@@ -1270,7 +1270,7 @@
   if (class_count_host[kNumClasses] > 0) {
     scratch_stride = ((int64_t)class_count_host[kNumClasses + 1] + 255) / 256 * 256;
     int64_t slices = class_count_host[kNumClasses];
-    if (4 * (int64_t)link_fixed_words(g->num_nodes, cn_cap, K) > 163840 || getenv("S3GRL_FORCE_EXT_BITMAPS")) {
+    if (4 * (int64_t)link_fixed_words(g, cn_cap, K) > kLdsBytes || getenv("S3GRL_FORCE_EXT_BITMAPS")) {
       bm_ext_words = (3 * words_for(g->num_nodes) + 63) / 64 * 64;
       scratch_stride += (int64_t)bm_ext_words * 4;
       gs_chunk = (int)std::min<int64_t>(slices, std::max<int64_t>(64, ((int64_t)1 << 29) / scratch_stride));
```

Result: faster. 17.84 million link pairs/s (median of 6 runs) (+2.2%).
